# JianCao92/speaker-diarization

Hardware: AMD Instinct MI355X
Metric: diarized audio throughput (CD gw/BIC + CL hi/BIC) (higher is better)
Workload: dtype f64

## Files before the change

### include/spkd.h

```cpp
#ifndef SPKD_H
#define SPKD_H

#include <stddef.h>
#include <stdint.h>

#ifdef __cplusplus
extern "C" {
#endif

#define SPKD_ABI_VERSION 2
#define SPKD_DIM 39
#define SPKD_REC 820

typedef enum {
    SPKD_OK = 0,
    SPKD_EINVAL = 1,
    SPKD_EHIP = 2,
    SPKD_ENONFINITE = 3,
    SPKD_EOVERFLOW = 4,
    SPKD_ENOMEM = 5
} spkd_status;

typedef enum { SPKD_BIC = 0, SPKD_GLR = 1, SPKD_KL2 = 2, SPKD_KL2_PINV = 3 } spkd_kind;


typedef struct spkd_ctx spkd_ctx;

int spkd_abi_version(void);

spkd_status spkd_create(int device, void *stream, spkd_ctx **out);
spkd_status spkd_create_on_stream(int device, void *stream, spkd_ctx **out);
void spkd_destroy(spkd_ctx *ctx);
const char *spkd_last_error(const spkd_ctx *ctx);
spkd_status spkd_sync(spkd_ctx *ctx);

spkd_status spkd_malloc(spkd_ctx *ctx, size_t bytes, void **d_ptr);
spkd_status spkd_free(spkd_ctx *ctx, void *d_ptr);
spkd_status spkd_memcpy_h2d(spkd_ctx *ctx, void *d_dst, const void *h_src, size_t bytes);
spkd_status spkd_memcpy_d2h(spkd_ctx *ctx, void *h_dst, const void *d_src, size_t bytes);
spkd_status spkd_memcpy_d2d(spkd_ctx *ctx, void *d_dst, const void *d_src, size_t bytes);

enum {
    SPKD_T_CALL = 0, SPKD_T_CHUNK_STATS, SPKD_T_REDUCE_SETS, SPKD_T_PAIR_TERMS,
    SPKD_T_CLUSTER_PREP, SPKD_T_MATRIX, SPKD_T_AHC, SPKD_T_GW, SPKD_T_SW, SPKD_N_TIMERS
};
spkd_status spkd_last_kernel_ms(spkd_ctx *ctx, int which, float *ms);

spkd_status spkd_last_gw_items(spkd_ctx *ctx, int64_t *items);

spkd_status spkd_set_stats(spkd_ctx *ctx, const float *d_frames, int64_t n_frames,
                           const int64_t *h_range_begin, const int64_t *h_range_end,
                           const int32_t *h_range_set, int64_t n_ranges,
                           int64_t n_sets, double *d_stats);

#define SPKD_WANT_GLR 1
#define SPKD_WANT_KL2 2
#define SPKD_WANT_KL2_PINV 4
spkd_status spkd_pair_terms(spkd_ctx *ctx, const double *d_stats,
                            const int32_t *h_idx_a, const int32_t *h_idx_b,
                            int64_t n_pairs, int flags, double *h_terms);

spkd_status spkd_distance_matrix(spkd_ctx *ctx, int kind, double lambdac,
                                 const double *d_stats, int64_t n, double *d_matrix);

spkd_status spkd_cluster_in(spkd_ctx *ctx, const double *d_stats, int64_t n, int kind,
                            double lambdac, double threshold, int32_t *h_label,
                            double *h_dist, int64_t dist_cap, int64_t *h_dist_off,
                            int64_t *h_n_done, int64_t *h_n_clusters);

spkd_status spkd_distance_rows(spkd_ctx *ctx, int variant, int kind, double lambdac,
                               const double *d_stats, int64_t n, int64_t row_begin, int64_t row_end,
                               double *d_rows, double *h_stat_max, double *h_stat_min);

typedef struct {
    int32_t kind;
    int32_t trace;
    double lambdac;
    double threshold;
    double winsize;
    double winstep;
    double deltaws;
    double rate;
} spkd_cd_params;

typedef struct {
    int32_t turn;
    int32_t coarse;
    int64_t seq;
    double start, i, d;
    int64_t n1, n2;
} spkd_cand_log;

int64_t spkd_gw_event_capacity(int64_t turn_len, double rate);
int64_t spkd_gw_event_capacity_p(int64_t turn_len, const spkd_cd_params *params);
spkd_status spkd_gw(spkd_ctx *ctx, const float *d_frames, int64_t n_frames,
                    const int64_t *h_turn_begin, const int64_t *h_turn_end, int64_t n_turns,
                    const spkd_cd_params *params, const int64_t *h_ev_off,
                    int32_t *h_n_win, double *h_win_maxd, int32_t *h_win_det,
                    double *h_det_start, double *h_det_maxi, double *h_det_d,
                    double *h_final_start,
                    spkd_cand_log *h_log, int64_t log_cap, int64_t *h_log_count);

spkd_status spkd_gw_ex(spkd_ctx *ctx, const float *d_frames, int64_t n_frames,
                       const int64_t *h_turn_begin, const int64_t *h_turn_end, int64_t n_turns,
                       const spkd_cd_params *params, const int64_t *h_ev_off, int check_capacity,
                       int32_t *h_n_win, double *h_win_maxd, int32_t *h_win_det,
                       double *h_det_start, double *h_det_maxi, double *h_det_d,
                       double *h_final_start,
                       spkd_cand_log *h_log, int64_t log_cap, int64_t *h_log_count);

spkd_status spkd_gw_fused(spkd_ctx *ctx, const float *d_frames, int64_t n_frames,
                          const int64_t *h_turn_begin, const int64_t *h_turn_end, int64_t n_turns,
                          const spkd_cd_params *params, const int64_t *h_ev_off, int check_capacity,
                          int32_t *h_n_win, double *h_win_maxd, int32_t *h_win_det,
                          double *h_det_start, double *h_det_maxi, double *h_det_d,
                          double *h_final_start, double *d_seg_stats,
                          spkd_cand_log *h_log, int64_t log_cap, int64_t *h_log_count);

spkd_status spkd_gather_stats(spkd_ctx *ctx, const double *d_src, int64_t n_src,
                              const int64_t *h_src_index, const int64_t *h_dst_index,
                              int64_t n, int64_t n_dst, double *d_dst);

int64_t spkd_sw_window_count(int64_t turn_len, double winsize, double winstep);
spkd_status spkd_sw(spkd_ctx *ctx, const float *d_frames, int64_t n_frames,
                    const int64_t *h_turn_begin, const int64_t *h_turn_end, int64_t n_turns,
                    const spkd_cd_params *params, const int64_t *h_d_off, double *h_d);

enum { SPKD_AHC_AUTO = 0, SPKD_AHC_MONO = 1, SPKD_AHC_WIDE = 2 };

typedef struct {
    int32_t variant;
    int32_t kind;
    int32_t max_spk;
    int32_t path;
    double lambdac;
    double threshold;
} spkd_ahc_params;

spkd_status spkd_ahc(spkd_ctx *ctx, const double *d_stats, const int64_t *h_seg_off,
                     int64_t n_problems, const spkd_ahc_params *params,
                     int32_t *h_n_merges, int32_t *h_merge_a, int32_t *h_merge_b,
                     double *h_merge_d, double *h_stat_max, double *h_stat_min);

spkd_status spkd_ahc_matrix(spkd_ctx *ctx, const double *d_stats, int64_t n, const spkd_ahc_params *params,
                            const double *d_matrix, double stat_max_in, double stat_min_in,
                            int32_t *h_n_merges, int32_t *h_merge_a, int32_t *h_merge_b,
                            double *h_merge_d, double *h_stat_max, double *h_stat_min);

typedef struct {
    int32_t sample_rate, frame_rate, window_width, n_fft, n_mel, n_cep;
    int32_t cms_left, cms_right;
    int32_t delta_width[2];
    float pre_emph;
    float delta_norm[2];
} spkd_mfcc_params;
spkd_status spkd_mfcc(spkd_ctx *ctx, const int16_t *d_pcm, int64_t n_samples,
                      const spkd_mfcc_params *params, const float *h_melfb, const float *h_dct,
                      const float *h_mean, const float *h_scale, const float *h_transform,
                      float *d_features, int64_t *h_n_frames);

typedef struct {
    int32_t n_kernels, n_states, dim;
    const float *mean;
    const float *inv_var;
    const float *log_norm;
    const int32_t *state_off;
    const int32_t *kernel;
    const float *log_weight;
} spkd_gmm_params;
spkd_status spkd_gmm_loglik(spkd_ctx *ctx, const float *d_features, int64_t n_frames,
                            const spkd_gmm_params *params, float *d_scores);

void spkd_py2_roundtrip(double *h_values, int64_t n);
spkd_status spkd_labels_from_merges(int64_t n, int64_t n_merges, const int32_t *h_a,
                                    const int32_t *h_b, int32_t *h_labels);
spkd_status spkd_labels_from_merges_batch(int64_t n_problems, const int64_t *h_seg_off,
                                          const int32_t *h_n_merges, const int32_t *h_a,
                                          const int32_t *h_b, int32_t *h_labels);

spkd_status spkd_count_flags(const int32_t *h_flags, const int64_t *h_off, const int32_t *h_n,
                             int64_t n_groups, int32_t *h_out);

spkd_status spkd_gw_lines(int64_t n_turns, const int64_t *h_off, const int32_t *h_n_det,
                          const double *h_det_start, const double *h_det_maxi,
                          const double *h_final_start, const double *h_turn_start_s,
                          const double *h_turn_end_s, const int64_t *h_turn_begin,
                          const int64_t *h_turn_end, double rate, int text_contract,
                          int64_t n_lines, double *h_times, int64_t *h_frame_b,
                          int64_t *h_frame_e, int64_t *h_index, int32_t *h_line_turn);

spkd_status spkd_vad_viterbi(int64_t n_frames, int32_t n_states, const float *h_scores,
                             int32_t n_words, const int32_t *h_word_state, const double *h_stay,
                             const double *h_exit, const double *h_enter, int64_t *h_tok_frame,
                             int32_t *h_tok_word, int64_t *h_n_tokens, double *h_score);

#ifdef __cplusplus
}
#endif
#endif
```

### speaker-diarization_amd/csrc/spkd_hip.hip

```cpp
#include <hip/hip_runtime.h>

#include <algorithm>
#include <cmath>
#include <cstdio>
#include <cstdlib>
#include <cstring>
#include <string>
#include <atomic>
#include <thread>
#include <vector>

#include "../../include/spkd.h"
#include "spkd_cd.hpp"
#include "spkd_cluster.hpp"
#include "spkd_device.hpp"
#include "spkd_stats.hpp"
#include "spkd_mfcc.hpp"
#include "spkd_vad.hpp"

using namespace spkd;

namespace {
constexpr int N_SLOTS = 36;
}

struct spkd_ctx {
    int device = 0;
    hipStream_t stream = nullptr;
    bool own_stream = false;
    bool gw_lds_ok = false;
    int gw_waves = 0;
    unsigned long long init_keys[2] = {0ull, ~0ull};
    int step_waves = 0;
    int step_partners = 0;
    int64_t last_gw_items = 0;
    std::string err;
    int* d_err = nullptr;
    unsigned long long* d_counter = nullptr;
    hipEvent_t ev0 = nullptr, ev1 = nullptr;
    float last_ms = 0.f;
    hipEvent_t ka[SPKD_N_TIMERS] = {}, kb[SPKD_N_TIMERS] = {};
    bool kused[SPKD_N_TIMERS] = {};
    float kms[SPKD_N_TIMERS] = {};
    void* slot[N_SLOTS] = {};
    size_t slot_bytes[N_SLOTS] = {};
    void* pinv_ws = nullptr;
    double* pinv_cur = nullptr;
};

namespace {

spkd_status fail(spkd_ctx* c, spkd_status s, const std::string& msg) {
    if (c) c->err = msg;
    return s;
}

#define HIPCHK(c, call)                                                              \
    do {                                                                             \
        hipError_t e_ = (call);                                                      \
        if (e_ != hipSuccess)                                                        \
            return fail((c), SPKD_EHIP, std::string(#call) + ": " + hipGetErrorString(e_)); \
    } while (0)

#define TRY(expr) do { const spkd_status s_ = (expr); if (s_ != SPKD_OK) return s_; } while (0)

spkd_status scratch(spkd_ctx* c, int slot, size_t bytes, void** out) {
    if (bytes == 0) bytes = 16;
    if (c->slot_bytes[slot] < bytes) {
        if (c->slot[slot]) HIPCHK(c, hipFree(c->slot[slot]));
        c->slot[slot] = nullptr;
        c->slot_bytes[slot] = 0;
        size_t want = bytes + bytes / 4;
        hipError_t e = hipMalloc(&c->slot[slot], want);
        if (e != hipSuccess) {
            want = bytes;
            e = hipMalloc(&c->slot[slot], want);
        }
        if (e != hipSuccess) return fail(c, SPKD_ENOMEM, "scratch allocation failed");
        c->slot_bytes[slot] = want;
    }
    *out = c->slot[slot];
    return SPKD_OK;
}

template <class T>
spkd_status upload(spkd_ctx* c, int slot, const T* h, size_t n, T** d) {
    void* p = nullptr;
    TRY(scratch(c, slot, n * sizeof(T), &p));
    if (n) HIPCHK(c, hipMemcpyAsync(p, h, n * sizeof(T), hipMemcpyHostToDevice, c->stream));
    *d = (T*)p;
    return SPKD_OK;
}

struct Call {
    spkd_ctx* const c;
    spkd_status opened;
    int herr = 0;
    bool drained = false;
    explicit Call(spkd_ctx* ctx) : c(ctx) { opened = open(); }
    ~Call() { if (!drained) (void)hipStreamSynchronize(c->stream); }
    spkd_status open() {
        HIPCHK(c, hipSetDevice(c->device));
        for (int i = 0; i < SPKD_N_TIMERS; ++i) c->kused[i] = false;
        HIPCHK(c, hipMemsetAsync(c->d_err, 0, sizeof(int), c->stream));
        HIPCHK(c, hipEventRecord(c->ev0, c->stream));
        return SPKD_OK;
    }

    spkd_status finish() {
        HIPCHK(c, hipEventRecord(c->ev1, c->stream));
        HIPCHK(c, hipMemcpyAsync(&herr, c->d_err, sizeof(int), hipMemcpyDeviceToHost, c->stream));
        HIPCHK(c, hipStreamSynchronize(c->stream));
        drained = true;
        HIPCHK(c, hipEventElapsedTime(&c->last_ms, c->ev0, c->ev1));
        c->kms[0] = c->last_ms;
        for (int i = 1; i < SPKD_N_TIMERS; ++i)
            if (c->kused[i]) HIPCHK(c, hipEventElapsedTime(&c->kms[i], c->ka[i], c->kb[i]));
        if (herr & ERR_SWEEP) return fail(c, SPKD_EHIP, "internal error: growing-window sweep order");
        if (herr & 4) return fail(c, SPKD_EOVERFLOW, "device scratch capacity exceeded");
        if (herr & ERR_DEGENERATE_MERGE) return fail(c, SPKD_EINVAL, "degenerate merge: a diagonal cell was the minimum");
        if (herr & ERR_NONFINITE) return fail(c, SPKD_ENONFINITE, "array must not contain infs or NaNs");
        return SPKD_OK;
    }
};

spkd_status use_kind(spkd_ctx* c, int kind, int* base) {
    c->pinv_cur = nullptr;
    *base = kind;
    if (kind != SPKD_KL2_PINV) return SPKD_OK;
    *base = SPKD_KL2;
    if (!c->pinv_ws) {
        if (hipMalloc(&c->pinv_ws, PINV_WS_BYTES) != hipSuccess) {
            c->pinv_ws = nullptr;
            return fail(c, SPKD_ENOMEM, "pinv workspace allocation failed");
        }
        HIPCHK(c, hipMemsetAsync(c->pinv_ws, 0, PINV_LOCK_BYTES, c->stream));
    }
    c->pinv_cur = (double*)c->pinv_ws;
    return SPKD_OK;
}

struct Timer {
    spkd_ctx* const c;
    const int idx;
    Timer(spkd_ctx* ctx, int i) : c(ctx), idx(i) { (void)hipEventRecord(c->ka[idx], c->stream); }
    ~Timer() { (void)hipEventRecord(c->kb[idx], c->stream); c->kused[idx] = true; }
};

enum {
    S_CHUNKS = 0, S_SETOFF, S_PARTIAL, S_IDXA, S_IDXB, S_TERMS, S_TURNS, S_SNAP, S_CAND,
    S_EV_I32A, S_EV_I32B, S_EV_D0, S_EV_D1, S_EV_D2, S_EV_D3, S_EV_D4, S_LOG,
    S_AHC_STATS, S_AHC_LD, S_AHC_AUX, S_AHC_MAT, S_AHC_MISC, S_AHC_OUT, S_AHC_OFF, S_AHC_PROB, S_AHC_PACKED, S_MFCC_TAB, S_MFCC_STATIC,
    S_STEP_EXM, S_STEP_PKM, S_STEP_MISC, S_GMM_TAB, S_GMM_IDX, S_COUNT
};
static_assert(S_COUNT <= N_SLOTS, "scratch slot table too small");

}

extern "C" {

int spkd_abi_version(void) { return SPKD_ABI_VERSION; }

static spkd_status create_ctx(int device, void* stream, bool borrow, spkd_ctx** out) {
    if (!out) return SPKD_EINVAL;
    *out = nullptr;
    int count = 0;
    if (hipGetDeviceCount(&count) != hipSuccess || device < 0 || device >= count) return SPKD_EHIP;
    spkd_ctx* c = new spkd_ctx();
    c->device = device;
    if (hipSetDevice(device) != hipSuccess) { delete c; return SPKD_EHIP; }
    if (borrow) {
        c->stream = (hipStream_t)stream;
    } else {
        if (hipStreamCreateWithFlags(&c->stream, hipStreamDefault) != hipSuccess) { delete c; return SPKD_EHIP; }
        c->own_stream = true;
    }
    if (hipMalloc(&c->d_err, sizeof(int)) != hipSuccess ||
        hipMalloc(&c->d_counter, 2 * sizeof(unsigned long long)) != hipSuccess ||
        hipEventCreate(&c->ev0) != hipSuccess || hipEventCreate(&c->ev1) != hipSuccess) {
        spkd_destroy(c);
        return SPKD_EHIP;
    }
    for (int i = 0; i < SPKD_N_TIMERS; ++i)
        if (hipEventCreate(&c->ka[i]) != hipSuccess || hipEventCreate(&c->kb[i]) != hipSuccess) {
            spkd_destroy(c);
            return SPKD_EHIP;
        }
    int lds_max = 0;
    c->gw_lds_ok = hipDeviceGetAttribute(&lds_max, hipDeviceAttributeMaxSharedMemoryPerBlock, device) == hipSuccess &&
                   Gw<4>::LDS_BYTES <= lds_max &&
                   hipFuncSetAttribute((const void*)k_gw<8>, hipFuncAttributeMaxDynamicSharedMemorySize, Gw<8>::LDS_BYTES) == hipSuccess &&
                   hipFuncSetAttribute((const void*)k_gw<4>, hipFuncAttributeMaxDynamicSharedMemorySize, Gw<4>::LDS_BYTES) == hipSuccess &&
                   hipFuncSetAttribute((const void*)k_gw<2>, hipFuncAttributeMaxDynamicSharedMemorySize, Gw<2>::LDS_BYTES) == hipSuccess &&
                   hipFuncSetAttribute((const void*)k_gw<1>, hipFuncAttributeMaxDynamicSharedMemorySize, Gw<1>::LDS_BYTES) == hipSuccess;
    if (const char* e = getenv("SPKD_GW_WAVES")) c->gw_waves = atoi(e);
    if (const char* e = getenv("SPKD_STEP_WAVES")) { const int v = atoi(e); c->step_waves = (v == 4 || v == 8) ? v : 0; }
    if (const char* e = getenv("SPKD_STEP_PARTNERS")) { const int v = atoi(e); c->step_partners = (v == 3 || v == 7 || v == 15) ? v : 0; }
    *out = c;
    return SPKD_OK;
}

spkd_status spkd_create(int device, void* stream, spkd_ctx** out) {
    return create_ctx(device, stream, stream != nullptr, out);
}

spkd_status spkd_create_on_stream(int device, void* stream, spkd_ctx** out) {
    return create_ctx(device, stream, true, out);
}

void spkd_destroy(spkd_ctx* c) {
    if (!c) return;
    (void)hipSetDevice(c->device);
    if (c->stream) (void)hipStreamSynchronize(c->stream);
    for (int i = 0; i < N_SLOTS; ++i)
        if (c->slot[i]) (void)hipFree(c->slot[i]);
    if (c->d_err) (void)hipFree(c->d_err);
    if (c->pinv_ws) (void)hipFree(c->pinv_ws);
    if (c->d_counter) (void)hipFree(c->d_counter);
    if (c->ev0) (void)hipEventDestroy(c->ev0);
    if (c->ev1) (void)hipEventDestroy(c->ev1);
    for (int i = 0; i < SPKD_N_TIMERS; ++i) {
        if (c->ka[i]) (void)hipEventDestroy(c->ka[i]);
        if (c->kb[i]) (void)hipEventDestroy(c->kb[i]);
    }
    if (c->own_stream && c->stream) (void)hipStreamDestroy(c->stream);
    delete c;
}

const char* spkd_last_error(const spkd_ctx* c) { return c ? c->err.c_str() : "null context"; }

spkd_status spkd_sync(spkd_ctx* c) {
    if (!c) return SPKD_EINVAL;
    HIPCHK(c, hipStreamSynchronize(c->stream));
    return SPKD_OK;
}

spkd_status spkd_malloc(spkd_ctx* c, size_t bytes, void** d_ptr) {
    if (!c || !d_ptr) return SPKD_EINVAL;
    HIPCHK(c, hipSetDevice(c->device));
    hipError_t e = hipMalloc(d_ptr, bytes ? bytes : 16);
    if (e != hipSuccess) return fail(c, SPKD_ENOMEM, hipGetErrorString(e));
    return SPKD_OK;
}

spkd_status spkd_free(spkd_ctx* c, void* d_ptr) {
    if (!c) return SPKD_EINVAL;
    HIPCHK(c, hipFree(d_ptr));
    return SPKD_OK;
}

spkd_status spkd_memcpy_h2d(spkd_ctx* c, void* d_dst, const void* h_src, size_t bytes) {
    if (!c) return SPKD_EINVAL;
    HIPCHK(c, hipMemcpyAsync(d_dst, h_src, bytes, hipMemcpyHostToDevice, c->stream));
    HIPCHK(c, hipStreamSynchronize(c->stream));
    return SPKD_OK;
}

spkd_status spkd_memcpy_d2h(spkd_ctx* c, void* h_dst, const void* d_src, size_t bytes) {
    if (!c) return SPKD_EINVAL;
    HIPCHK(c, hipMemcpyAsync(h_dst, d_src, bytes, hipMemcpyDeviceToHost, c->stream));
    HIPCHK(c, hipStreamSynchronize(c->stream));
    return SPKD_OK;
}

spkd_status spkd_memcpy_d2d(spkd_ctx* c, void* d_dst, const void* d_src, size_t bytes) {
    if (!c) return SPKD_EINVAL;
    HIPCHK(c, hipMemcpyAsync(d_dst, d_src, bytes, hipMemcpyDeviceToDevice, c->stream));
    HIPCHK(c, hipStreamSynchronize(c->stream));
    return SPKD_OK;
}

spkd_status spkd_last_gw_items(spkd_ctx* c, int64_t* items) {
    if (!c || !items) return SPKD_EINVAL;
    *items = c->last_gw_items;
    return SPKD_OK;
}

spkd_status spkd_last_kernel_ms(spkd_ctx* c, int which, float* ms) {
    if (!c || !ms || which < 0 || which >= SPKD_N_TIMERS) return SPKD_EINVAL;
    *ms = c->kms[which];
    return SPKD_OK;
}

namespace {
spkd_status set_stats_launch(spkd_ctx* c, const float* d_frames, int64_t n_frames,
                             const int64_t* h_begin, const int64_t* h_end, const int32_t* h_set,
                             int64_t n_ranges, int64_t n_sets, double* d_stats,
                             std::vector<Chunk>& chunks, std::vector<int64_t>& set_off) {
    chunks.clear();
    set_off.assign((size_t)n_sets + 1, 0);
    int32_t prev = 0;
    for (int64_t r = 0; r < n_ranges; ++r) {
        const int64_t b = h_begin[r], e = h_end[r];
        const int32_t s = h_set[r];
        if (b < 0 || e < b || e > n_frames || s < prev || s >= n_sets)
            return fail(c, SPKD_EINVAL, "bad frame range or set id");
        prev = s;
        for (int64_t t = b; t < e; t += STATS_CHUNK) {
            Chunk ch;
            ch.begin = t;
            ch.len = (int32_t)std::min<int64_t>(STATS_CHUNK, e - t);
            ch.set = s;
            chunks.push_back(ch);
            set_off[(size_t)s + 1]++;
        }
    }
    for (int64_t s = 0; s < n_sets; ++s) set_off[(size_t)s + 1] += set_off[(size_t)s];
    Chunk* d_chunks = nullptr;
    int64_t* d_setoff = nullptr;
    void* d_partial = nullptr;
    TRY(upload(c, S_CHUNKS, chunks.data(), chunks.size(), &d_chunks));
    TRY(upload(c, S_SETOFF, set_off.data(), set_off.size(), &d_setoff));
    TRY(scratch(c, S_PARTIAL, chunks.size() * REC * sizeof(double), &d_partial));
    if (!chunks.empty()) {
        Timer t(c, SPKD_T_CHUNK_STATS);
        hipLaunchKernelGGL(k_chunk_stats, dim3((unsigned)chunks.size()), dim3(STATS_TPB), 0, c->stream,
                           d_frames, d_chunks, (double*)d_partial);
    }
    Timer t(c, SPKD_T_REDUCE_SETS);
    hipLaunchKernelGGL(k_reduce_sets, dim3((unsigned)n_sets), dim3(STATS_TPB), 0, c->stream,
                       (const double*)d_partial, d_setoff, d_stats);
    HIPCHK(c, hipGetLastError());
    return SPKD_OK;
}
}

spkd_status spkd_set_stats(spkd_ctx* c, const float* d_frames, int64_t n_frames,
                           const int64_t* h_begin, const int64_t* h_end, const int32_t* h_set,
                           int64_t n_ranges, int64_t n_sets, double* d_stats) {
    if (!c || !d_stats || n_sets < 0 || n_ranges < 0) return SPKD_EINVAL;
    if (n_sets == 0) return SPKD_OK;
    if (n_ranges > 0 && (!h_begin || !h_end || !h_set || !d_frames)) return fail(c, SPKD_EINVAL, "null range arrays");
    std::vector<Chunk> chunks;
    std::vector<int64_t> set_off;
    Call call(c);
    TRY(call.opened);
    TRY(set_stats_launch(c, d_frames, n_frames, h_begin, h_end, h_set, n_ranges, n_sets, d_stats, chunks, set_off));
    return call.finish();
}

spkd_status spkd_pair_terms(spkd_ctx* c, const double* d_stats, const int32_t* h_a, const int32_t* h_b,
                            int64_t n_pairs, int flags, double* h_terms) {
    if (!c || n_pairs < 0) return SPKD_EINVAL;
    if (n_pairs == 0) return SPKD_OK;
    if (!d_stats || !h_a || !h_b || !h_terms) return fail(c, SPKD_EINVAL, "null argument");
    if ((flags & SPKD_WANT_KL2) && (flags & SPKD_WANT_KL2_PINV))
        return fail(c, SPKD_EINVAL, "pair_terms: SPKD_WANT_KL2 and SPKD_WANT_KL2_PINV exclude each other");
    Call call(c);
    TRY(call.opened);
    int kind_unused;
    TRY(use_kind(c, (flags & SPKD_WANT_KL2_PINV) ? (int)SPKD_KL2_PINV : (int)SPKD_KL2, &kind_unused));
    if (flags & SPKD_WANT_KL2_PINV) flags = (flags & ~SPKD_WANT_KL2_PINV) | SPKD_WANT_KL2;
    int32_t *d_a = nullptr, *d_b = nullptr;
    void* d_terms = nullptr;
    TRY(upload(c, S_IDXA, h_a, (size_t)n_pairs, &d_a));
    TRY(upload(c, S_IDXB, h_b, (size_t)n_pairs, &d_b));
    TRY(scratch(c, S_TERMS, (size_t)n_pairs * 8 * sizeof(double), &d_terms));
    const unsigned blocks = (unsigned)((n_pairs + PT2_WAVES - 1) / PT2_WAVES);
    {
        Timer t(c, SPKD_T_PAIR_TERMS);
        hipLaunchKernelGGL(k_pair_terms, dim3(blocks), dim3(PT2_WAVES * WAVE), 0, c->stream,
                           d_stats, d_a, d_b, n_pairs, flags, (double*)d_terms, c->d_err, c->pinv_cur);
    }
    HIPCHK(c, hipGetLastError());
    HIPCHK(c, hipMemcpyAsync(h_terms, d_terms, (size_t)n_pairs * 8 * sizeof(double), hipMemcpyDeviceToHost, c->stream));
    return call.finish();
}

namespace {
struct AhcBuffers {
    double* ex;
    double* pk;
    double* ld;
    double* aux;
    double* mat;
    int64_t* seg_off;
    int64_t* mat_off;
    unsigned long long* smax;
    unsigned long long* smin;
};

unsigned long long host_dkey(double v) {
    unsigned long long b;
    std::memcpy(&b, &v, sizeof b);
    return (b >> 63) ? ~b : (b | 0x8000000000000000ull);
}

struct MatrixPlan {
    const double* d_init = nullptr;
    double init_max = NAN, init_min = NAN;
    int64_t row_begin = -1, row_end = -1;
};

spkd_status ahc_prepare(spkd_ctx* c, const double* d_stats, const int64_t* h_seg_off, int64_t n_prob,
                        int variant, int kind, double lambdac, AhcBuffers& B, int64_t& n_total,
                        std::vector<int64_t>& offs, std::vector<int32_t>& prob_of,
                        const MatrixPlan& plan = MatrixPlan()) {
    n_total = h_seg_off[n_prob];
    offs.clear();
    offs.insert(offs.end(), h_seg_off, h_seg_off + n_prob + 1);
    int64_t cells = 0;
    for (int64_t p = 0; p < n_prob; ++p) {
        const int64_t n = h_seg_off[p + 1] - h_seg_off[p];
        if (n < 0) return fail(c, SPKD_EINVAL, "seg_off must be non-decreasing");
        offs.push_back(cells);
        cells += n * n;
    }
    offs.push_back(cells);
    prob_of.assign((size_t)n_total, 0);
    for (int64_t p = 0; p < n_prob; ++p)
        for (int64_t r = h_seg_off[p]; r < h_seg_off[p + 1]; ++r) prob_of[(size_t)r] = (int32_t)p;
    int64_t grid_rows = 0;
    {
        const int X = 8;
        std::vector<std::vector<int32_t>> lists(X);
        if (plan.row_begin >= 0) {
            for (int64_t r = plan.row_begin; r < plan.row_end; ++r) lists[(size_t)((r - plan.row_begin) % X)].push_back((int32_t)r);
        } else if (n_prob >= X) {
            std::vector<int64_t> order((size_t)n_prob);
            for (int64_t p = 0; p < n_prob; ++p) order[(size_t)p] = p;
            std::stable_sort(order.begin(), order.end(), [&](int64_t a, int64_t b) {
                return h_seg_off[a + 1] - h_seg_off[a] > h_seg_off[b + 1] - h_seg_off[b];
            });
            double load[X] = {0, 0, 0, 0, 0, 0, 0, 0};
            for (int64_t p : order) {
                int x = 0;
                for (int i = 1; i < X; ++i) if (load[i] < load[x]) x = i;
                const double n = (double)(h_seg_off[p + 1] - h_seg_off[p]);
                load[x] += n * n;
                for (int64_t r = h_seg_off[p]; r < h_seg_off[p + 1]; ++r) lists[x].push_back((int32_t)r);
            }
        } else {
            for (int64_t r = 0; r < n_total; ++r) lists[(size_t)(r % X)].push_back((int32_t)r);
        }
        size_t longest = 0;
        for (auto& l : lists) longest = std::max(longest, l.size());
        grid_rows = (int64_t)longest * X;
        prob_of.resize((size_t)(n_total + grid_rows), -1);
        for (int x = 0; x < X; ++x)
            for (size_t i = 0; i < lists[x].size(); ++i) prob_of[(size_t)n_total + i * X + x] = lists[x][i];
    }
    int64_t* d_offs = nullptr;
    int32_t* d_prob = nullptr;
    TRY(upload(c, S_AHC_OFF, offs.data(), offs.size(), &d_offs));
    TRY(upload(c, S_AHC_PROB, prob_of.data(), prob_of.size(), &d_prob));
    B.seg_off = d_offs;
    B.mat_off = d_offs + n_prob + 1;
    void* p = nullptr;
    TRY(scratch(c, S_AHC_LD, (size_t)n_total * sizeof(double), &p));
    B.ld = (double*)p;
    TRY(scratch(c, S_AHC_AUX, (size_t)n_total * AUX * sizeof(double), &p));
    B.aux = (double*)p;
    TRY(scratch(c, S_AHC_MAT, (size_t)cells * sizeof(double), &p));
    B.mat = (double*)p;
    TRY(scratch(c, S_AHC_MISC, (size_t)n_prob * 2 * sizeof(unsigned long long), &p));
    B.smax = (unsigned long long*)p;
    B.smin = B.smax + n_prob;
    HIPCHK(c, hipMemsetAsync(B.smax, 0x00, (size_t)n_prob * sizeof(unsigned long long), c->stream));
    HIPCHK(c, hipMemsetAsync(B.smin, 0xff, (size_t)n_prob * sizeof(unsigned long long), c->stream));
    if (plan.d_init && n_prob == 1) {
        c->init_keys[0] = plan.init_max == plan.init_max ? host_dkey(plan.init_max) : 0ull;
        c->init_keys[1] = plan.init_min == plan.init_min ? host_dkey(plan.init_min) : ~0ull;
        HIPCHK(c, hipMemcpyAsync(B.smax, &c->init_keys[0], sizeof(unsigned long long), hipMemcpyHostToDevice, c->stream));
        HIPCHK(c, hipMemcpyAsync(B.smin, &c->init_keys[1], sizeof(unsigned long long), hipMemcpyHostToDevice, c->stream));
    }
    TRY(scratch(c, S_AHC_STATS, (size_t)n_total * QREC * sizeof(double), &p));
    B.ex = (double*)p;
    TRY(scratch(c, S_AHC_PACKED, (size_t)n_total * REC * sizeof(double), &p));
    B.pk = (double*)p;
    if (n_total > 0) {
        hipLaunchKernelGGL(k_to_quadrec, dim3((unsigned)n_total), dim3(256), 0, c->stream, d_stats, n_total, B.ex);
        HIPCHK(c, hipMemcpyAsync(B.pk, d_stats, (size_t)n_total * REC * sizeof(double), hipMemcpyDeviceToDevice, c->stream));
        const int64_t per_block = kind == SPKD_KL2 ? PT_WAVES : 4 * PT_WAVES;
        const unsigned blocks = (unsigned)((n_total + per_block - 1) / per_block);
        {
            Timer t(c, SPKD_T_CLUSTER_PREP);
            hipLaunchKernelGGL(k_cluster_prep, dim3(blocks), dim3(PT_WAVES * WAVE), 0, c->stream,
                               (const double*)B.ex, n_total, kind, B.ld, B.aux, c->d_err, c->pinv_cur);
        }
        auto kmat = kind == SPKD_GLR ? k_matrix<true> : k_matrix<false>;
        if (plan.d_init) {
            HIPCHK(c, hipMemcpyAsync(B.mat, plan.d_init, (size_t)cells * sizeof(double), hipMemcpyDeviceToDevice, c->stream));
        } else if (grid_rows > 0) {
            Timer t(c, SPKD_T_MATRIX);
            hipLaunchKernelGGL(kmat, dim3((unsigned)grid_rows), dim3(MX_WAVES * WAVE), 0, c->stream,
                               (const double*)B.ex, (const double*)B.pk, (const int64_t*)B.seg_off, (const int32_t*)d_prob,
                               (const int32_t*)d_prob + n_total, variant, kind, lambdac,
                               (const double*)B.ld, (const double*)B.aux, B.mat, (const int64_t*)B.mat_off,
                               B.smax, B.smin, c->d_err);
        }
    }
    HIPCHK(c, hipGetLastError());
    return SPKD_OK;
}

double key_to_double(unsigned long long k, bool is_max) {
    if (is_max ? (k == 0ull) : (k == ~0ull)) return std::nan("");
    unsigned long long b = (k >> 63) ? (k & 0x7fffffffffffffffull) : ~k;
    double v;
    std::memcpy(&v, &b, sizeof v);
    return v;
}
}

spkd_status spkd_distance_matrix(spkd_ctx* c, int kind, double lambdac, const double* d_stats,
                                 int64_t n, double* d_matrix) {
    if (!c || n < 0 || kind < 0 || kind > 3) return SPKD_EINVAL;
    if (n == 0) return SPKD_OK;
    if (!d_stats || !d_matrix) return fail(c, SPKD_EINVAL, "null argument");
    const int64_t seg_off[2] = {0, n};
    AhcBuffers B;
    int64_t n_total = 0;
    std::vector<int64_t> offs;
    std::vector<int32_t> prob_of;
    Call call(c);
    TRY(call.opened);
    TRY(use_kind(c, kind, &kind));
    TRY(ahc_prepare(c, d_stats, seg_off, 1, 1, kind, lambdac, B, n_total, offs, prob_of));
    HIPCHK(c, hipMemcpyAsync(d_matrix, B.mat, (size_t)n * n * sizeof(double), hipMemcpyDeviceToDevice, c->stream));
    return call.finish();
}

spkd_status spkd_cluster_in(spkd_ctx* c, const double* d_stats, int64_t n, int kind, double lambdac, double threshold,
                            int32_t* h_label, double* h_dist, int64_t dist_cap, int64_t* h_dist_off,
                            int64_t* h_n_done, int64_t* h_n_clusters) {
    if (!c || n < 0 || dist_cap < 0 || kind < 0 || kind > 3) return SPKD_EINVAL;
    if (h_n_done) *h_n_done = 0;
    if (h_n_clusters) *h_n_clusters = 0;
    if (n == 0) return SPKD_OK;
    if (!d_stats || !h_label || !h_dist_off || !h_n_done || !h_n_clusters || (dist_cap > 0 && !h_dist))
        return fail(c, SPKD_EINVAL, "null argument");
    long long done2[2] = {0, 0};
    Call call(c);
    TRY(call.opened);
    TRY(use_kind(c, kind, &kind));
    void *p_ex = nullptr, *p_ld = nullptr, *p_aux = nullptr, *p_cex = nullptr, *p_cpk = nullptr, *p_misc = nullptr, *p_dist = nullptr;
    const size_t nn = (size_t)n;
    TRY(scratch(c, S_AHC_STATS, nn * QREC * sizeof(double), &p_ex));
    TRY(scratch(c, S_AHC_LD, nn * sizeof(double), &p_ld));
    TRY(scratch(c, S_AHC_AUX, nn * AUX * sizeof(double), &p_aux));
    TRY(scratch(c, S_STEP_EXM, nn * QREC * sizeof(double), &p_cex));
    TRY(scratch(c, S_STEP_PKM, nn * REC * sizeof(double), &p_cpk));
    const size_t misc_bytes = (2 + AUX) * nn * sizeof(double) + (nn + 1 + 2) * sizeof(long long) + nn * sizeof(int32_t) + 64;
    TRY(scratch(c, S_STEP_MISC, misc_bytes, &p_misc));
    TRY(scratch(c, S_AHC_MAT, (size_t)std::max<int64_t>(dist_cap, 1) * sizeof(double), &p_dist));
    double* clu_ld = (double*)p_misc;
    double* tmp = clu_ld + nn;
    double* clu_aux = tmp + nn;
    long long* d_off = (long long*)(clu_aux + nn * AUX);
    long long* d_done = d_off + nn + 1;
    int32_t* d_label = (int32_t*)(d_done + 2);
    HIPCHK(c, hipMemsetAsync(d_done, 0, 2 * sizeof(long long), c->stream));
    hipLaunchKernelGGL(k_to_quadrec, dim3((unsigned)n), dim3(256), 0, c->stream, d_stats, n, (double*)p_ex);
    {
        const int64_t per_block = 4 * PT_WAVES;
        const unsigned blocks = (unsigned)((n + per_block - 1) / per_block);
        {
            Timer t(c, SPKD_T_CLUSTER_PREP);
            hipLaunchKernelGGL(k_cluster_prep, dim3(blocks), dim3(PT_WAVES * WAVE), 0, c->stream,
                               (const double*)p_ex, n, kind == SPKD_KL2 ? (int)SPKD_BIC : kind, (double*)p_ld, (double*)p_aux, c->d_err,
                               c->pinv_cur);
        }
        if (kind == SPKD_KL2) {
            void* p_ld2 = nullptr;
            TRY(scratch(c, S_AHC_OUT, nn * sizeof(double), &p_ld2));
            const unsigned blocks1 = (unsigned)((n + PT_WAVES - 1) / PT_WAVES);
            hipLaunchKernelGGL(k_cluster_prep, dim3(blocks1), dim3(PT_WAVES * WAVE), 0, c->stream,
                               (const double*)p_ex, n, (int)SPKD_KL2, (double*)p_ld2, (double*)p_aux, c->d_err, c->pinv_cur);
        }
    }
    auto kin = kind == SPKD_GLR ? k_cluster_in<true> : k_cluster_in<false>;
    {
        Timer t(c, SPKD_T_AHC);
        hipLaunchKernelGGL(kin, dim3(1), dim3(CIN_TPB), 0, c->stream,
                           (const double*)p_ex, d_stats, (const double*)p_ld, (const double*)p_aux, (long long)n, kind, lambdac, threshold,
                           (double*)p_cex, (double*)p_cpk, clu_ld, clu_aux, tmp, d_label, (double*)p_dist, (long long)dist_cap,
                           d_off, d_done, c->d_err, c->pinv_cur);
    }
    HIPCHK(c, hipGetLastError());
    HIPCHK(c, hipMemcpyAsync(done2, d_done, sizeof done2, hipMemcpyDeviceToHost, c->stream));
    HIPCHK(c, hipMemcpyAsync(h_label, d_label, nn * sizeof(int32_t), hipMemcpyDeviceToHost, c->stream));
    HIPCHK(c, hipMemcpyAsync(h_dist_off, d_off, (nn + 1) * sizeof(long long), hipMemcpyDeviceToHost, c->stream));
    if (dist_cap > 0)
        HIPCHK(c, hipMemcpyAsync(h_dist, p_dist, (size_t)dist_cap * sizeof(double), hipMemcpyDeviceToHost, c->stream));
    const spkd_status st = call.finish();
    *h_n_done = done2[0];
    *h_n_clusters = done2[1];
    return st;
}

spkd_status spkd_distance_rows(spkd_ctx* c, int variant, int kind, double lambdac, const double* d_stats,
                               int64_t n, int64_t row_begin, int64_t row_end, double* d_rows,
                               double* h_stat_max, double* h_stat_min) {
    if (!c || n < 0 || kind < 0 || kind > 3 || (variant != 1 && variant != 2)) return SPKD_EINVAL;
    if (row_begin < 0 || row_end < row_begin || row_end > n) return fail(c, SPKD_EINVAL, "distance_rows: bad row block");
    if (h_stat_max) *h_stat_max = std::nan("");
    if (h_stat_min) *h_stat_min = std::nan("");
    if (n == 0 || row_end == row_begin) return SPKD_OK;
    if (!d_stats || !d_rows) return fail(c, SPKD_EINVAL, "null argument");
    const int64_t seg_off[2] = {0, n};
    AhcBuffers B;
    int64_t n_total = 0;
    std::vector<int64_t> offs;
    std::vector<int32_t> prob_of;
    MatrixPlan plan;
    plan.row_begin = row_begin;
    plan.row_end = row_end;
    unsigned long long keys[2] = {0ull, ~0ull};
    Call call(c);
    TRY(call.opened);
    TRY(use_kind(c, kind, &kind));
    TRY(ahc_prepare(c, d_stats, seg_off, 1, variant, kind, lambdac, B, n_total, offs, prob_of, plan));
    HIPCHK(c, hipMemcpyAsync(d_rows, B.mat + row_begin * n, (size_t)(row_end - row_begin) * n * sizeof(double),
                             hipMemcpyDeviceToDevice, c->stream));
    HIPCHK(c, hipMemcpyAsync(&keys[0], B.smax, sizeof(unsigned long long), hipMemcpyDeviceToHost, c->stream));
    HIPCHK(c, hipMemcpyAsync(&keys[1], B.smin, sizeof(unsigned long long), hipMemcpyDeviceToHost, c->stream));
    const spkd_status st = call.finish();
    if (h_stat_max) *h_stat_max = key_to_double(keys[0], true);
    if (h_stat_min) *h_stat_min = key_to_double(keys[1], false);
    return st;
}

namespace {
spkd_status ahc_impl(spkd_ctx* c, const double* d_stats, const int64_t* h_seg_off, int64_t n_prob,
                     const spkd_ahc_params* P, const MatrixPlan& plan, int32_t* h_n_merges, int32_t* h_merge_a,
                     int32_t* h_merge_b, double* h_merge_d, double* h_stat_max, double* h_stat_min) {
    if (!c || !P || n_prob < 0) return SPKD_EINVAL;
    if (n_prob == 0) return SPKD_OK;
    if (!d_stats || !h_seg_off || !h_n_merges || !h_merge_a || !h_merge_b || !h_merge_d ||
        !h_stat_max || !h_stat_min)
        return fail(c, SPKD_EINVAL, "null argument");
    if ((P->variant != 1 && P->variant != 2) || P->kind < 0 || P->kind > 3)
        return fail(c, SPKD_EINVAL, "bad variant / kind");
    for (int64_t p = 0; p < n_prob; ++p)
        if (h_seg_off[p + 1] - h_seg_off[p] < 1) return fail(c, SPKD_EINVAL, "empty clustering problem");
    int64_t n_max = 0;
    for (int64_t p = 0; p < n_prob; ++p) n_max = std::max<int64_t>(n_max, h_seg_off[p + 1] - h_seg_off[p]);
    if (n_max > AHC_MAX_N) return fail(c, SPKD_EINVAL, "clustering problem larger than 65536 records");
    int path = P->path;
    if (path != SPKD_AHC_MONO && path != SPKD_AHC_WIDE) path = n_prob <= 64 ? SPKD_AHC_WIDE : SPKD_AHC_MONO;
    const size_t lds = (size_t)(n_max + 4) * sizeof(int32_t);
    if (path == SPKD_AHC_MONO && lds > 150 * 1024) path = SPKD_AHC_WIDE;
    if (path == SPKD_AHC_WIDE && n_max > STEP_MAX_N)
        return fail(c, SPKD_EINVAL, "clustering problem larger than 16384 records (wide merge loop)");
    AhcBuffers B;
    int64_t n_total = 0;
    std::vector<int64_t> offs;
    std::vector<int32_t> prob_of;
    std::vector<unsigned long long> kmax((size_t)n_prob), kmin((size_t)n_prob);
    std::vector<double> fmax((size_t)n_prob), fmin((size_t)n_prob);
    Call call(c);
    TRY(call.opened);
    spkd_ahc_params Pk = *P;
    TRY(use_kind(c, P->kind, &Pk.kind));
    P = &Pk;
    TRY(ahc_prepare(c, d_stats, h_seg_off, n_prob, P->variant, P->kind, P->lambdac, B, n_total, offs, prob_of, plan));
    void* op = nullptr;
    const size_t out_bytes = (size_t)n_total * (6 * sizeof(int32_t) + 3 * sizeof(double)) +
                             (size_t)n_prob * (sizeof(int32_t) + 2 * sizeof(double)) + 64;
    TRY(scratch(c, S_AHC_OUT, out_bytes, &op));
    double* d_merge_d = (double*)op;
    double* d_tmp = d_merge_d + n_total;
    double* d_rmin = d_tmp + n_total;
    double* d_fmax = d_rmin + n_total;
    double* d_fmin = d_fmax + n_prob;
    int32_t* d_a = (int32_t*)(d_fmin + n_prob);
    int32_t* d_b = d_a + n_total;
    int32_t* d_alive = d_b + n_total;
    int32_t* d_rcache = d_alive + n_total;
    int32_t* d_n = d_rcache + 3 * n_total;
    if (path == SPKD_AHC_MONO) {
        auto kahc = P->kind == SPKD_GLR ? k_ahc<true> : k_ahc<false>;
        if (lds > 48 * 1024)
            (void)hipFuncSetAttribute((const void*)kahc, hipFuncAttributeMaxDynamicSharedMemorySize, (int)lds);
        Timer t(c, SPKD_T_AHC);
        hipLaunchKernelGGL(kahc, dim3((unsigned)n_prob), dim3(AHC_TPB), lds, c->stream,
                           B.ex, B.pk, (const int64_t*)B.seg_off, P->variant, P->kind, P->max_spk, P->lambdac,
                           P->threshold, B.ld, B.aux, B.mat, (const int64_t*)B.mat_off, d_alive, d_tmp,
                           d_rmin, d_rcache, d_n, d_a, d_b, d_merge_d, B.smax, B.smin, d_fmax, d_fmin, c->d_err,
                           c->pinv_cur);
    } else {
        StepArrays Q;
        void *pm = nullptr, *pe = nullptr, *pp = nullptr;
        const size_t nt = (size_t)n_total;
        const size_t misc_bytes = nt * 2 * sizeof(StepSel) + nt * sizeof(double) + nt * sizeof(unsigned long long) +
                                  (size_t)2 * n_prob * sizeof(StepState) + nt * sizeof(int32_t) + 64;
        TRY(scratch(c, S_STEP_MISC, misc_bytes, &pm));
        TRY(scratch(c, S_STEP_EXM, nt * QREC * sizeof(double), &pe));
        TRY(scratch(c, S_STEP_PKM, nt * REC * sizeof(double), &pp));
        Q.ex = B.ex; Q.pk = B.pk; Q.exm = (double*)pe; Q.pkm = (double*)pp;
        Q.sel2 = (StepSel*)pm;
        Q.cnt = (double*)(Q.sel2 + 2 * nt);
        Q.sw = (unsigned long long*)(Q.cnt + nt);
        Q.state2 = (StepState*)(Q.sw + nt);
        Q.death = (int32_t*)(Q.state2 + 2 * n_prob);
        Q.n_total = n_total;
        Q.n_prob = (int32_t)n_prob;
        const int step_waves = c->step_waves ? c->step_waves : (n_max > STEP_WIDE_FROM ? 8 : 4);
        const bool glr_k = P->kind == SPKD_GLR;
        using StepKernel = decltype(&k_ahc_step<false, 4, 3>);
        StepKernel kvar[3];
        if (step_waves == 8) {
            kvar[0] = glr_k ? k_ahc_step<true, 8, 3> : k_ahc_step<false, 8, 3>;
            kvar[1] = glr_k ? k_ahc_step<true, 8, 7> : k_ahc_step<false, 8, 7>;
            kvar[2] = glr_k ? k_ahc_step<true, 8, STEP_PARTNERS> : k_ahc_step<false, 8, STEP_PARTNERS>;
        } else {
            kvar[0] = glr_k ? k_ahc_step<true, 4, 3> : k_ahc_step<false, 4, 3>;
            kvar[1] = glr_k ? k_ahc_step<true, 4, 7> : k_ahc_step<false, 4, 7>;
            kvar[2] = glr_k ? k_ahc_step<true, 4, STEP_PARTNERS> : k_ahc_step<false, 4, STEP_PARTNERS>;
        }
        auto sp_of_round = [&](int64_t partners) -> int {
            if (c->step_partners) return c->step_partners;
            const int64_t free_cus = 255;
            if (partners * n_prob <= 3 * free_cus) return 3;
            if (partners * n_prob <= 7 * free_cus) return 7;
            return STEP_PARTNERS;
        };
        const size_t nch_max = (size_t)((n_max + WAVE - 1) / WAVE);
        const size_t step_lds = ((size_t)2 * n_max + nch_max + 2) * sizeof(int32_t) + nch_max * sizeof(unsigned long long);
        if (step_lds + 20 * 1024 > 48 * 1024)
            for (int v = 0; v < 3; ++v)
                (void)hipFuncSetAttribute((const void*)kvar[v], hipFuncAttributeMaxDynamicSharedMemorySize, (int)step_lds);
        Timer t(c, SPKD_T_AHC);
        const unsigned row_blocks = (unsigned)((n_max + AHC_WAVES - 1) / AHC_WAVES);
        hipLaunchKernelGGL(k_step_init, dim3(row_blocks, (unsigned)n_prob), dim3(AHC_TPB), 0, c->stream,
                           (const int64_t*)B.seg_off, (const double*)B.mat, (const int64_t*)B.mat_off, Q);
        for (int64_t it = 1; it < n_max; ++it) {
            const int64_t partners = n_max - it - 1;
            const int step_sp = sp_of_round(partners);
            StepKernel kstep = kvar[step_sp == 3 ? 0 : (step_sp == 7 ? 1 : 2)];
            const unsigned blocks = (unsigned)std::max<int64_t>(1, (partners + step_sp - 1) / step_sp) + 1;
            hipLaunchKernelGGL(kstep, dim3(blocks, (unsigned)n_prob), dim3(step_waves * WAVE), step_lds, c->stream,
                               (int)it, (const int64_t*)B.seg_off, P->variant, P->kind, P->max_spk, P->lambdac,
                               P->threshold, B.ld, B.aux, B.mat, (const int64_t*)B.mat_off, Q, d_a, d_b, d_merge_d,
                               B.smax, B.smin, c->d_err, c->pinv_cur);
        }
        hipLaunchKernelGGL(k_step_final, dim3((unsigned)n_prob), dim3(AHC_TPB), 0, c->stream,
                           (int)(n_max - 1), (const int64_t*)B.seg_off, (const double*)B.mat, (const int64_t*)B.mat_off,
                           Q, d_n, d_fmax, d_fmin);
    }
    HIPCHK(c, hipGetLastError());
    HIPCHK(c, hipMemcpyAsync(h_n_merges, d_n, (size_t)n_prob * sizeof(int32_t), hipMemcpyDeviceToHost, c->stream));
    HIPCHK(c, hipMemcpyAsync(h_merge_a, d_a, (size_t)n_total * sizeof(int32_t), hipMemcpyDeviceToHost, c->stream));
    HIPCHK(c, hipMemcpyAsync(h_merge_b, d_b, (size_t)n_total * sizeof(int32_t), hipMemcpyDeviceToHost, c->stream));
    HIPCHK(c, hipMemcpyAsync(h_merge_d, d_merge_d, (size_t)n_total * sizeof(double), hipMemcpyDeviceToHost, c->stream));
    HIPCHK(c, hipMemcpyAsync(kmax.data(), B.smax, (size_t)n_prob * sizeof(unsigned long long), hipMemcpyDeviceToHost, c->stream));
    HIPCHK(c, hipMemcpyAsync(kmin.data(), B.smin, (size_t)n_prob * sizeof(unsigned long long), hipMemcpyDeviceToHost, c->stream));
    HIPCHK(c, hipMemcpyAsync(fmax.data(), d_fmax, (size_t)n_prob * sizeof(double), hipMemcpyDeviceToHost, c->stream));
    HIPCHK(c, hipMemcpyAsync(fmin.data(), d_fmin, (size_t)n_prob * sizeof(double), hipMemcpyDeviceToHost, c->stream));
    const spkd_status st = call.finish();
    for (int64_t p = 0; p < n_prob; ++p) {
        if (P->variant == 1) {
            h_stat_max[p] = key_to_double(kmax[(size_t)p], true);
            h_stat_min[p] = key_to_double(kmin[(size_t)p], false);
        } else {
            h_stat_max[p] = fmax[(size_t)p];
            h_stat_min[p] = fmin[(size_t)p];
        }
    }
    return st;
}
}

spkd_status spkd_ahc(spkd_ctx* c, const double* d_stats, const int64_t* h_seg_off, int64_t n_prob,
                     const spkd_ahc_params* P, int32_t* h_n_merges, int32_t* h_merge_a,
                     int32_t* h_merge_b, double* h_merge_d, double* h_stat_max, double* h_stat_min) {
    return ahc_impl(c, d_stats, h_seg_off, n_prob, P, MatrixPlan(), h_n_merges, h_merge_a, h_merge_b, h_merge_d,
                    h_stat_max, h_stat_min);
}

spkd_status spkd_ahc_matrix(spkd_ctx* c, const double* d_stats, int64_t n, const spkd_ahc_params* P,
                            const double* d_matrix, double stat_max_in, double stat_min_in,
                            int32_t* h_n_merges, int32_t* h_merge_a, int32_t* h_merge_b, double* h_merge_d,
                            double* h_stat_max, double* h_stat_min) {
    if (!c || n < 1) return SPKD_EINVAL;
    if (!d_matrix) return fail(c, SPKD_EINVAL, "ahc_matrix: null matrix");
    const int64_t seg_off[2] = {0, n};
    MatrixPlan plan;
    plan.d_init = d_matrix;
    plan.init_max = stat_max_in;
    plan.init_min = stat_min_in;
    return ahc_impl(c, d_stats, seg_off, 1, P, plan, h_n_merges, h_merge_a, h_merge_b, h_merge_d, h_stat_max, h_stat_min);
}

int64_t spkd_gw_event_capacity(int64_t turn_len, double rate) {
    if (turn_len < 0 || !(rate >= 10.0)) return -1;
    return (int64_t)((double)turn_len / (0.2 * rate)) + 8;
}

int64_t spkd_gw_event_capacity_p(int64_t turn_len, const spkd_cd_params* P) {
    if (turn_len < 0 || !P || !(P->rate >= 10.0) || !(P->winstep >= 1.0)) return -1;
    const double step = std::min(0.2 * P->rate, std::min(0.5 * P->rate, P->winstep));
    return (int64_t)((double)turn_len / step) + 8;
}

int64_t spkd_sw_window_count(int64_t turn_len, double winsize, double winstep) {
    if (!(winstep >= 1.0) || !(winsize >= 1.0)) return -1;
    int64_t w = 0;
    for (double s = 0; s + 2 * winsize <= (double)turn_len; s += winstep) ++w;
    return w;
}

namespace {
spkd_status build_turns(spkd_ctx* c, int64_t n_frames, const int64_t* hb, const int64_t* he, int64_t n_turns,
                        const spkd_cd_params* P, const int64_t* h_off, bool gw, std::vector<TurnDesc>& turns,
                        int64_t& n_cand) {
    n_cand = 0;
    turns.resize((size_t)n_turns);
    for (int64_t t = 0; t < n_turns; ++t) {
        if (hb[t] < 0 || he[t] < hb[t] || he[t] > n_frames) return fail(c, SPKD_EINVAL, "bad turn range");
        TurnDesc& T = turns[(size_t)t];
        T.begin = hb[t];
        T.len = he[t] - hb[t];
        T.cand_off = n_cand;
        T.cand_cap = gw ? (int64_t)((double)T.len / (P->rate / 10)) + (int64_t)(2 * (P->rate / 10)) + 16 : 0;
        n_cand += T.cand_cap;
        T.ev_off = h_off[t];
        T.ev_cap = h_off[t + 1] - h_off[t];
        T.id = t;
        if (T.ev_cap < 0) return fail(c, SPKD_EINVAL, "offsets must be non-decreasing");
    }
    if (gw) std::stable_sort(turns.begin(), turns.end(), [](const TurnDesc& a, const TurnDesc& b) { return a.len > b.len; });
    return SPKD_OK;
}
}

namespace {
constexpr int64_t GW_WAVE_PER_TURN_FROM = 4096;
constexpr int64_t GW_EIGHT_WAVES_UP_TO = 256;
spkd_status gw_impl(spkd_ctx* c, const float* d_frames, int64_t n_frames, const int64_t* hb,
                    const int64_t* he, int64_t n_turns, const spkd_cd_params* P, const int64_t* h_ev_off,
                    int check_capacity, int32_t* h_n_win, double* h_win_maxd, int32_t* h_win_det,
                    double* h_det_start, double* h_det_maxi, double* h_det_d, double* h_final_start,
                    double* d_seg_stats, spkd_cand_log* h_log, int64_t log_cap, int64_t* h_log_count) {
    if (!c || !P || n_turns < 0) return SPKD_EINVAL;
    if (h_log_count) *h_log_count = 0;
    if (n_turns == 0) return SPKD_OK;
    if (!d_frames || !hb || !he || !h_ev_off || !h_n_win || !h_win_maxd || !h_win_det || !h_det_start ||
        !h_det_maxi || !h_det_d || !h_final_start)
        return fail(c, SPKD_EINVAL, "null argument");
    if (P->kind < 0 || P->kind > 3) return fail(c, SPKD_EINVAL, "gw: bad kind");
    if (!(P->rate >= 10.0) || !(P->winsize >= 1.0) || !(P->winstep >= 1.0))
        return fail(c, SPKD_EINVAL, "gw: rate >= 10, winsize >= 1 frame and winstep >= 1 frame required");
    if (log_cap < 0 || (log_cap > 0 && !h_log)) return fail(c, SPKD_EINVAL, "gw: log capacity without a log buffer");
    if (!c->gw_lds_ok) return fail(c, SPKD_EHIP, "gw: the kernel's dynamic LDS size was not admitted on this device");
    std::vector<TurnDesc> turns;
    int64_t n_cand;
    TRY(build_turns(c, n_frames, hb, he, n_turns, P, h_ev_off, true, turns, n_cand));
    for (int64_t t = 0; check_capacity && t < n_turns; ++t)
        if (turns[(size_t)t].ev_cap < spkd_gw_event_capacity_p(turns[(size_t)t].len, P))
            return fail(c, SPKD_EINVAL, "gw: event capacity too small, see spkd_gw_event_capacity_p");
    unsigned long long cnt2[2] = {0ull, 0ull};
    Call call(c);
    TRY(call.opened);
    spkd_cd_params Pk = *P;
    TRY(use_kind(c, P->kind, &Pk.kind));
    P = &Pk;
    const int64_t n_ev = h_ev_off[n_turns];
    TurnDesc* d_turns = nullptr;
    void *d_snap = nullptr, *d_cand = nullptr, *d_i32a = nullptr, *d_i32b = nullptr, *d_d0 = nullptr, *d_d1 = nullptr,
         *d_d2 = nullptr, *d_d3 = nullptr, *d_d4 = nullptr, *d_log = nullptr;
    TRY(upload(c, S_TURNS, turns.data(), turns.size(), &d_turns));
    TRY(scratch(c, S_SNAP, (size_t)n_cand * REC * sizeof(double), &d_snap));
    TRY(scratch(c, S_CAND, (size_t)n_cand * 4 * sizeof(double), &d_cand));
    TRY(scratch(c, S_EV_I32A, (size_t)n_turns * sizeof(int32_t), &d_i32a));
    TRY(scratch(c, S_EV_I32B, (size_t)n_ev * sizeof(int32_t), &d_i32b));
    TRY(scratch(c, S_EV_D0, (size_t)n_ev * sizeof(double), &d_d0));
    TRY(scratch(c, S_EV_D1, (size_t)n_ev * sizeof(double), &d_d1));
    TRY(scratch(c, S_EV_D2, (size_t)n_ev * sizeof(double), &d_d2));
    TRY(scratch(c, S_EV_D3, (size_t)n_ev * sizeof(double), &d_d3));
    TRY(scratch(c, S_EV_D4, (size_t)n_turns * sizeof(double), &d_d4));
    TRY(scratch(c, S_LOG, (size_t)std::max<int64_t>(log_cap, 1) * sizeof(spkd_cand_log), &d_log));
    if (!d_turns || !d_snap || !d_cand || !d_i32a || !d_i32b || !d_d0 || !d_d1 || !d_d2 || !d_d3 || !d_d4 ||
        !d_log || !c->d_counter || !c->d_err)
        return fail(c, SPKD_EHIP, "gw: a device scratch buffer is missing");
    HIPCHK(c, hipMemsetAsync(c->d_counter, 0, 2 * sizeof(unsigned long long), c->stream));
    int nw = c->gw_waves;
    if (nw != 1 && nw != 2 && nw != 4 && nw != 8)
        nw = n_turns >= GW_WAVE_PER_TURN_FROM ? 1 : (n_turns <= GW_EIGHT_WAVES_UP_TO ? 8 : 4);
#define SPKD_GW_LAUNCH(NW_)                                                                                     \
    hipLaunchKernelGGL(k_gw<NW_>, dim3((unsigned)n_turns), dim3(Gw<NW_>::TPB), Gw<NW_>::LDS_BYTES, c->stream, \
                       d_frames, (const TurnDesc*)d_turns, *P, (double*)d_snap, (double*)d_cand,               \
                       (int32_t*)d_i32a, (double*)d_d0, (int32_t*)d_i32b, (double*)d_d1, (double*)d_d2,        \
                       (double*)d_d3, (double*)d_d4, d_seg_stats, (spkd_cand_log*)d_log, (long long)log_cap,   \
                       c->d_counter, c->d_err, c->pinv_cur)
    {
        Timer t(c, SPKD_T_GW);
        if (nw == 1) SPKD_GW_LAUNCH(1); else if (nw == 2) SPKD_GW_LAUNCH(2);
        else if (nw == 8) SPKD_GW_LAUNCH(8); else SPKD_GW_LAUNCH(4);
    }
#undef SPKD_GW_LAUNCH
    HIPCHK(c, hipGetLastError());
    unsigned long long& cnt = cnt2[0];
    HIPCHK(c, hipMemcpyAsync(h_n_win, d_i32a, (size_t)n_turns * sizeof(int32_t), hipMemcpyDeviceToHost, c->stream));
    HIPCHK(c, hipMemcpyAsync(h_win_maxd, d_d0, (size_t)n_ev * sizeof(double), hipMemcpyDeviceToHost, c->stream));
    HIPCHK(c, hipMemcpyAsync(h_win_det, d_i32b, (size_t)n_ev * sizeof(int32_t), hipMemcpyDeviceToHost, c->stream));
    HIPCHK(c, hipMemcpyAsync(h_det_start, d_d1, (size_t)n_ev * sizeof(double), hipMemcpyDeviceToHost, c->stream));
    HIPCHK(c, hipMemcpyAsync(h_det_maxi, d_d2, (size_t)n_ev * sizeof(double), hipMemcpyDeviceToHost, c->stream));
    HIPCHK(c, hipMemcpyAsync(h_det_d, d_d3, (size_t)n_ev * sizeof(double), hipMemcpyDeviceToHost, c->stream));
    HIPCHK(c, hipMemcpyAsync(h_final_start, d_d4, (size_t)n_turns * sizeof(double), hipMemcpyDeviceToHost, c->stream));
    HIPCHK(c, hipMemcpyAsync(cnt2, c->d_counter, sizeof cnt2, hipMemcpyDeviceToHost, c->stream));
    const spkd_status st = call.finish();
    c->last_gw_items = (int64_t)cnt2[1];
    if (h_log_count) *h_log_count = (int64_t)cnt;
    if (h_log && log_cap > 0 && cnt > 0) {
        const size_t ncopy = (size_t)std::min<int64_t>((int64_t)cnt, log_cap);
        HIPCHK(c, hipMemcpy(h_log, d_log, ncopy * sizeof(spkd_cand_log), hipMemcpyDeviceToHost));
    }
    if (st == SPKD_OK && (int64_t)cnt > log_cap && h_log)
        return fail(c, SPKD_EOVERFLOW, "candidate log too small");
    return st;
}
}

spkd_status spkd_gw(spkd_ctx* c, const float* d_frames, int64_t n_frames, const int64_t* hb,
                    const int64_t* he, int64_t n_turns, const spkd_cd_params* P, const int64_t* h_ev_off,
                    int32_t* h_n_win, double* h_win_maxd, int32_t* h_win_det, double* h_det_start,
                    double* h_det_maxi, double* h_det_d, double* h_final_start, spkd_cand_log* h_log,
                    int64_t log_cap, int64_t* h_log_count) {
    return gw_impl(c, d_frames, n_frames, hb, he, n_turns, P, h_ev_off, 1, h_n_win, h_win_maxd, h_win_det,
                   h_det_start, h_det_maxi, h_det_d, h_final_start, nullptr, h_log, log_cap, h_log_count);
}

spkd_status spkd_gw_ex(spkd_ctx* c, const float* d_frames, int64_t n_frames, const int64_t* hb,
                       const int64_t* he, int64_t n_turns, const spkd_cd_params* P, const int64_t* h_ev_off,
                       int check_capacity, int32_t* h_n_win, double* h_win_maxd, int32_t* h_win_det,
                       double* h_det_start, double* h_det_maxi, double* h_det_d, double* h_final_start,
                       spkd_cand_log* h_log, int64_t log_cap, int64_t* h_log_count) {
    return gw_impl(c, d_frames, n_frames, hb, he, n_turns, P, h_ev_off, check_capacity, h_n_win, h_win_maxd,
                   h_win_det, h_det_start, h_det_maxi, h_det_d, h_final_start, nullptr, h_log, log_cap,
                   h_log_count);
}

spkd_status spkd_gw_fused(spkd_ctx* c, const float* d_frames, int64_t n_frames, const int64_t* hb,
                          const int64_t* he, int64_t n_turns, const spkd_cd_params* P, const int64_t* h_ev_off,
                          int check_capacity, int32_t* h_n_win, double* h_win_maxd, int32_t* h_win_det,
                          double* h_det_start, double* h_det_maxi, double* h_det_d, double* h_final_start,
                          double* d_seg_stats, spkd_cand_log* h_log, int64_t log_cap, int64_t* h_log_count) {
    if (c && !d_seg_stats) return fail(c, SPKD_EINVAL, "gw_fused: null statistics buffer");
    return gw_impl(c, d_frames, n_frames, hb, he, n_turns, P, h_ev_off, check_capacity, h_n_win, h_win_maxd,
                   h_win_det, h_det_start, h_det_maxi, h_det_d, h_final_start, d_seg_stats, h_log, log_cap,
                   h_log_count);
}

namespace {
__global__ __launch_bounds__(256) void k_gather_records(const double* __restrict__ src, const int64_t* __restrict__ si,
                                                        const int64_t* __restrict__ di, int64_t n,
                                                        double* __restrict__ dst) {
    const int64_t i = blockIdx.x;
    if (i >= n) return;
    const double2* s = reinterpret_cast<const double2*>(src + si[i] * REC);
    double2* d = reinterpret_cast<double2*>(dst + (di ? di[i] : i) * REC);
    for (int e = threadIdx.x; e < REC / 2; e += 256) d[e] = s[e];
}
}

spkd_status spkd_gather_stats(spkd_ctx* c, const double* d_src, int64_t n_src, const int64_t* h_src_index,
                              const int64_t* h_dst_index, int64_t n, int64_t n_dst, double* d_dst) {
    if (!c || n < 0) return SPKD_EINVAL;
    if (n == 0) return SPKD_OK;
    if (!d_src || !h_src_index || !d_dst) return fail(c, SPKD_EINVAL, "null argument");
    for (int64_t i = 0; i < n; ++i) {
        if (h_src_index[i] < 0 || h_src_index[i] >= n_src) return fail(c, SPKD_EINVAL, "gather: source index out of range");
        const int64_t d = h_dst_index ? h_dst_index[i] : i;
        if (d < 0 || d >= n_dst) return fail(c, SPKD_EINVAL, "gather: destination index out of range");
    }
    Call call(c);
    TRY(call.opened);
    int64_t *d_si = nullptr, *d_di = nullptr;
    TRY(upload(c, S_IDXA, h_src_index, (size_t)n, &d_si));
    if (h_dst_index) TRY(upload(c, S_IDXB, h_dst_index, (size_t)n, &d_di));
    hipLaunchKernelGGL(k_gather_records, dim3((unsigned)n), dim3(256), 0, c->stream, d_src,
                       (const int64_t*)d_si, (const int64_t*)d_di, n, d_dst);
    HIPCHK(c, hipGetLastError());
    return call.finish();
}

namespace {
__global__ __launch_bounds__(256) void k_take_pair_distance(const double* __restrict__ mat, int64_t n, double* __restrict__ out) {
    const int64_t p = (int64_t)blockIdx.x * 256 + threadIdx.x;
    if (p < n) out[p] = mat[4 * p + 1];
}
}

spkd_status spkd_sw(spkd_ctx* c, const float* d_frames, int64_t n_frames, const int64_t* hb,
                    const int64_t* he, int64_t n_turns, const spkd_cd_params* P, const int64_t* h_d_off,
                    double* h_d) {
    if (!c || !P || n_turns < 0) return SPKD_EINVAL;
    if (n_turns == 0) return SPKD_OK;
    if (!d_frames || !hb || !he || !h_d_off || !h_d) return fail(c, SPKD_EINVAL, "null argument");
    if (P->kind < 0 || P->kind > 3) return fail(c, SPKD_EINVAL, "bad kind");
    if (!(P->winsize >= 1.0) || !(P->winstep >= 1.0)) return fail(c, SPKD_EINVAL, "sw: window and step must be >= 1 frame");
    const int64_t n_d = h_d_off[n_turns];
    std::vector<int64_t> rb, re;
    std::vector<int32_t> rs;
    rb.reserve((size_t)(2 * n_d)); re.reserve((size_t)(2 * n_d)); rs.reserve((size_t)(2 * n_d));
    const int64_t wsz = (int64_t)P->winsize;
    for (int64_t t = 0; t < n_turns; ++t) {
        if (hb[t] < 0 || he[t] < hb[t] || he[t] > n_frames) return fail(c, SPKD_EINVAL, "bad turn range");
        const int64_t len = he[t] - hb[t];
        const int64_t W = spkd_sw_window_count(len, P->winsize, P->winstep);
        if (h_d_off[t + 1] - h_d_off[t] != W) return fail(c, SPKD_EINVAL, "sw: offsets do not match spkd_sw_window_count");
        for (int64_t w = 0; w < W; ++w) {
            const int64_t a = hb[t] + (int64_t)((double)w * P->winstep);
            const int32_t s0 = (int32_t)(2 * (h_d_off[t] + w));
            rb.push_back(a); re.push_back(a + wsz); rs.push_back(s0);
            rb.push_back(a + wsz); re.push_back(a + 2 * wsz); rs.push_back(s0 + 1);
        }
    }
    if (n_d == 0) return SPKD_OK;
    if (2 * n_d > 0x7fffffffLL) return fail(c, SPKD_EINVAL, "sw: too many windows in one call");
    std::vector<Chunk> chunks;
    std::vector<int64_t> set_off, offs;
    std::vector<int32_t> prob_of;
    Call call(c);
    TRY(call.opened);
    spkd_cd_params Pk = *P;
    TRY(use_kind(c, P->kind, &Pk.kind));
    P = &Pk;
    void *d_rec = nullptr, *d_out = nullptr;
    TRY(scratch(c, S_SNAP, (size_t)(2 * n_d) * REC * sizeof(double), &d_rec));
    TRY(scratch(c, S_EV_D0, (size_t)n_d * sizeof(double), &d_out));
    {
        Timer t(c, SPKD_T_SW);
        TRY(set_stats_launch(c, d_frames, n_frames, rb.data(), re.data(), rs.data(), 2 * n_d, 2 * n_d, (double*)d_rec,
                             chunks, set_off));
        std::vector<int64_t> seg_off((size_t)n_d + 1);
        for (int64_t w = 0; w <= n_d; ++w) seg_off[(size_t)w] = 2 * w;
        AhcBuffers B;
        int64_t n_total = 0;
        TRY(ahc_prepare(c, (const double*)d_rec, seg_off.data(), n_d, 1, P->kind, P->lambdac, B, n_total, offs, prob_of));
        hipLaunchKernelGGL(k_take_pair_distance, dim3((unsigned)((n_d + 255) / 256)), dim3(256), 0, c->stream,
                           (const double*)B.mat, n_d, (double*)d_out);
    }
    HIPCHK(c, hipGetLastError());
    HIPCHK(c, hipMemcpyAsync(h_d, d_out, (size_t)n_d * sizeof(double), hipMemcpyDeviceToHost, c->stream));
    return call.finish();
}

spkd_status spkd_mfcc(spkd_ctx* c, const int16_t* d_pcm, int64_t n_samples, const spkd_mfcc_params* P,
                      const float* h_melfb, const float* h_dct, const float* h_mean, const float* h_scale,
                      const float* h_transform, float* d_features, int64_t* h_n_frames) {
    if (!c || !P || !h_n_frames) return SPKD_EINVAL;
    *h_n_frames = 0;
    if (n_samples < 0 || !h_melfb || !h_dct || !h_mean || !h_scale || !h_transform)
        return fail(c, SPKD_EINVAL, "mfcc: null argument");
    if ((P->window_width != MF_WIN && P->window_width != MF_WIN_VAD) || P->n_fft != MF_NFFT || P->n_mel != MF_MEL ||
        P->n_cep != MF_CEP || P->frame_rate <= 0 || P->sample_rate <= 0 || P->sample_rate % P->frame_rate != 0)
        return fail(c, SPKD_EINVAL, "mfcc: this build does 400- or 256-sample windows, a 512-point transform, 21 mel bins, 12 cepstra");
    if (P->cms_left < 0 || P->cms_right < 0 || P->cms_left + P->cms_right > 1024 || P->delta_width[0] < 1 ||
        P->delta_width[0] > 2 || P->delta_width[1] < 1 || P->delta_width[1] > 2 || !(P->delta_norm[0] > 0.f) ||
        !(P->delta_norm[1] > 0.f))
        return fail(c, SPKD_EINVAL, "mfcc: unsupported mean-subtraction window or delta parameters");
    const int hop = P->sample_rate / P->frame_rate;
    if (hop < 1) return fail(c, SPKD_EINVAL, "mfcc: frame rate above the sample rate");
    const int span = MP_FR + 2 * MP_HALO;
    const size_t lds = (size_t)((span + P->cms_left + P->cms_right) * MF_STATIC + 2 * span * MF_STATIC +
                                MP_FR * MF_DIM + MF_DIM * MF_DIM) * sizeof(float);
    if (lds > 60 * 1024) return fail(c, SPKD_EINVAL, "mfcc: mean-subtraction window too wide for the LDS tile");
    const int64_t T = n_samples / hop;
    *h_n_frames = T;
    if (T == 0) return SPKD_OK;
    if (!d_pcm || !d_features) return fail(c, SPKD_EINVAL, "mfcc: null device buffer");
    std::vector<float> tab;
    tab.insert(tab.end(), h_melfb, h_melfb + MF_MEL * MF_BINS);
    tab.insert(tab.end(), h_dct, h_dct + MF_CEP * MF_MEL);
    tab.insert(tab.end(), h_mean, h_mean + MF_DIM);
    tab.insert(tab.end(), h_scale, h_scale + MF_DIM);
    tab.insert(tab.end(), h_transform, h_transform + MF_DIM * MF_DIM);
    Call call(c);
    TRY(call.opened);
    float* d_tab = nullptr;
    void* d_static = nullptr;
    TRY(upload(c, S_MFCC_TAB, tab.data(), tab.size(), &d_tab));
    TRY(scratch(c, S_MFCC_STATIC, (size_t)T * MF_STATIC * sizeof(float), &d_static));
    const float* d_fb = d_tab;
    const float* d_dct = d_fb + MF_MEL * MF_BINS;
    const float* d_mean = d_dct + MF_CEP * MF_MEL;
    const float* d_scale = d_mean + MF_DIM;
    const float* d_tr = d_scale + MF_DIM;
    if (P->window_width == MF_WIN)
        hipLaunchKernelGGL(k_mfcc_static<MF_WIN>, dim3((unsigned)((T + MF_FR - 1) / MF_FR)), dim3(MF_TPB), 0, c->stream,
                           d_pcm, (long long)n_samples, (long long)T, hop, P->pre_emph, d_fb, d_dct, (float*)d_static);
    else
        hipLaunchKernelGGL(k_mfcc_static<MF_WIN_VAD>, dim3((unsigned)((T + MF_FR - 1) / MF_FR)), dim3(MF_TPB), 0,
                           c->stream, d_pcm, (long long)n_samples, (long long)T, hop, P->pre_emph, d_fb, d_dct,
                           (float*)d_static);
    hipLaunchKernelGGL(k_mfcc_post, dim3((unsigned)((T + MP_FR - 1) / MP_FR)), dim3(MF_TPB), lds, c->stream,
                       (const float*)d_static, (long long)T, P->cms_left, P->cms_right, P->delta_width[0],
                       P->delta_norm[0], P->delta_width[1], P->delta_norm[1], d_mean, d_scale, d_tr, d_features);
    if (hipGetLastError() != hipSuccess) return fail(c, SPKD_EHIP, "mfcc: kernel launch failed");
    return call.finish();
}

spkd_status spkd_gmm_loglik(spkd_ctx* c, const float* d_features, int64_t n_frames, const spkd_gmm_params* P,
                            float* d_scores) {
    if (!c || !P) return SPKD_EINVAL;
    const int K = P->n_kernels, S = P->n_states;
    if (P->dim != GM_DIM || K < 1 || K > GM_MAX_K || S < 1 || S > GM_MAX_S || n_frames < 0)
        return fail(c, SPKD_EINVAL, "gmm_loglik: dim must be 39, 1 <= kernels <= 256, 1 <= states <= 16");
    if (!P->mean || !P->inv_var || !P->log_norm || !P->state_off || !P->kernel || !P->log_weight)
        return fail(c, SPKD_EINVAL, "gmm_loglik: null model array");
    if (P->state_off[0] != 0) return fail(c, SPKD_EINVAL, "gmm_loglik: state_off[0] must be 0");
    for (int s = 0; s < S; ++s)
        if (P->state_off[s + 1] < P->state_off[s] || P->state_off[s + 1] - P->state_off[s] > K)
            return fail(c, SPKD_EINVAL, "gmm_loglik: state_off must be non-decreasing, at most 256 kernels a state");
    const int nnz = P->state_off[S];
    for (int j = 0; j < nnz; ++j) {
        const float lw = P->log_weight[j];
        if (P->kernel[j] < 0 || P->kernel[j] >= K || std::isnan(lw) || lw == INFINITY)
            return fail(c, SPKD_EINVAL, "gmm_loglik: kernel index out of range or log weight NaN / +inf");
    }
    for (int64_t i = 0; i < (int64_t)K * GM_DIM; ++i)
        if (!std::isfinite(P->mean[i]) || !std::isfinite(P->inv_var[i]) || !(P->inv_var[i] > 0.f))
            return fail(c, SPKD_EINVAL, "gmm_loglik: means must be finite, inverse variances finite and positive");
    for (int k = 0; k < K; ++k)
        if (!std::isfinite(P->log_norm[k])) return fail(c, SPKD_EINVAL, "gmm_loglik: non-finite normalising constant");
    if (n_frames == 0) return SPKD_OK;
    if (!d_features || !d_scores) return fail(c, SPKD_EINVAL, "gmm_loglik: null device buffer");
    const int64_t n_blocks = (n_frames + GM_TPB - 1) / GM_TPB;
    if (n_blocks > 0x7fffffffLL) return fail(c, SPKD_EINVAL, "gmm_loglik: too many frames in one call");
    std::vector<float> tab;
    tab.insert(tab.end(), P->mean, P->mean + (size_t)K * GM_DIM);
    tab.insert(tab.end(), P->inv_var, P->inv_var + (size_t)K * GM_DIM);
    tab.insert(tab.end(), P->log_norm, P->log_norm + K);
    tab.insert(tab.end(), P->log_weight, P->log_weight + nnz);
    std::vector<int32_t> idx(P->state_off, P->state_off + S + 1);
    idx.insert(idx.end(), P->kernel, P->kernel + nnz);
    Call call(c);
    TRY(call.opened);
    float* d_tab = nullptr;
    int32_t* d_idx = nullptr;
    TRY(upload(c, S_GMM_TAB, tab.data(), tab.size(), &d_tab));
    TRY(upload(c, S_GMM_IDX, idx.data(), idx.size(), &d_idx));
    const float* d_mean = d_tab;
    const float* d_iv = d_mean + (size_t)K * GM_DIM;
    const float* d_c = d_iv + (size_t)K * GM_DIM;
    const float* d_lw = d_c + K;
    hipLaunchKernelGGL(k_gmm_loglik, dim3((unsigned)n_blocks), dim3(GM_TPB), 0, c->stream, d_features,
                       (long long)n_frames, d_mean, d_iv, d_c, (const int*)d_idx, (const int*)(d_idx + S + 1), d_lw,
                       S, d_scores);
    if (hipGetLastError() != hipSuccess) return fail(c, SPKD_EHIP, "gmm_loglik: kernel launch failed");
    return call.finish();
}

static const double kPow10[23] = {1e0, 1e1, 1e2, 1e3, 1e4, 1e5, 1e6, 1e7, 1e8, 1e9, 1e10, 1e11,
                                  1e12, 1e13, 1e14, 1e15, 1e16, 1e17, 1e18, 1e19, 1e20, 1e21, 1e22};
static const uint64_t kPow10u[20] = {1ull, 10ull, 100ull, 1000ull, 10000ull, 100000ull, 1000000ull,
                                     10000000ull, 100000000ull, 1000000000ull, 10000000000ull,
                                     100000000000ull, 1000000000000ull, 10000000000000ull,
                                     100000000000000ull, 1000000000000000ull, 10000000000000000ull,
                                     100000000000000000ull, 1000000000000000000ull,
                                     10000000000000000000ull};

static bool roundtrip_fast(double x, double* out) {
    if (!(x >= 1e-3 && x < 1e11)) return false;
    int e10 = (int)std::floor(std::log10(x));
    if (e10 < -3) e10 = -3;
    if (e10 >= 0) { if (x < kPow10[e10]) --e10; else if (e10 + 1 <= 22 && x >= kPow10[e10 + 1]) ++e10; }
    else { if (x * kPow10[-e10] < 1.0) --e10; else if (x * kPow10[-e10 - 1] >= 1.0) ++e10; }
    if (e10 < -3 || e10 > 10) return false;
    int s = 11 - e10;
    int k;
    const double fr = std::frexp(x, &k);
    const uint64_t m = (uint64_t)std::ldexp(fr, 53);
    k -= 53;
    unsigned __int128 prod = (unsigned __int128)m * kPow10u[s];
    uint64_t q;
    if (k >= 0) {
        if (k > 20) return false;
        q = (uint64_t)(prod << k);
    } else {
        const int sh = -k;
        if (sh >= 120) return false;
        const unsigned __int128 one = 1;
        const unsigned __int128 fl = prod >> sh;
        const unsigned __int128 remn = prod & ((one << sh) - 1);
        const unsigned __int128 half = one << (sh - 1);
        q = (uint64_t)fl;
        if (remn > half || (remn == half && (q & 1))) ++q;
    }
    if (q >= 1000000000000ull) {
        if (q != 1000000000000ull) return false;
        q = 100000000000ull;
        s -= 1;
    } else if (q < 100000000000ull) {
        return false;
    }
    *out = s >= 0 ? (double)q / kPow10[s] : (double)q * kPow10[-s];
    return true;
}

static void roundtrip_range(double* v, int64_t lo, int64_t hi) {
    char buf[64];
    for (int64_t i = lo; i < hi; ++i) {
        double r;
        if (roundtrip_fast(v[i], &r)) { v[i] = r; continue; }
        std::snprintf(buf, sizeof buf, "%.12g", v[i]);
        v[i] = std::strtod(buf, nullptr);
    }
}

void spkd_py2_roundtrip(double* v, int64_t n) {
    const int64_t kMinPerThread = 8192;
    int nthreads = (int)std::min<int64_t>(8, n / kMinPerThread);
    if (nthreads <= 1) { roundtrip_range(v, 0, n); return; }
    std::vector<std::thread> pool;
    const int64_t step = (n + nthreads - 1) / nthreads;
    for (int t = 0; t < nthreads; ++t) {
        const int64_t lo = t * step, hi = std::min<int64_t>(n, lo + step);
        if (lo < hi) pool.emplace_back(roundtrip_range, v, lo, hi);
    }
    for (auto& th : pool) th.join();
}

spkd_status spkd_labels_from_merges(int64_t n, int64_t n_merges, const int32_t* h_a, const int32_t* h_b,
                                    int32_t* h_labels) {
    if (n < 0 || n_merges < 0 || (n > 0 && !h_labels) || (n_merges > 0 && (!h_a || !h_b))) return SPKD_EINVAL;
    std::vector<int32_t> ids((size_t)n), parent((size_t)n);
    for (int64_t i = 0; i < n; ++i) ids[(size_t)i] = parent[(size_t)i] = (int32_t)i;
    int64_t m = n;
    for (int64_t k = 0; k < n_merges; ++k) {
        const int32_t a = h_a[k], b = h_b[k];
        if (a < 0 || b <= a || b >= m) return SPKD_EINVAL;
        parent[(size_t)ids[(size_t)b]] = ids[(size_t)a];
        ids.erase(ids.begin() + b);
        --m;
    }
    std::vector<int32_t> where((size_t)n, -1);
    for (int64_t p = 0; p < m; ++p) where[(size_t)ids[(size_t)p]] = (int32_t)p;
    for (int64_t i = 0; i < n; ++i) {
        int32_t r = (int32_t)i;
        while (parent[(size_t)r] != r) r = parent[(size_t)r];
        int32_t c = (int32_t)i;
        while (parent[(size_t)c] != r) { const int32_t nx = parent[(size_t)c]; parent[(size_t)c] = r; c = nx; }
        h_labels[i] = where[(size_t)r] + 1;
    }
    return SPKD_OK;
}

spkd_status spkd_count_flags(const int32_t* h_flags, const int64_t* h_off, const int32_t* h_n, int64_t n_groups,
                             int32_t* h_out) {
    if (n_groups < 0 || (n_groups > 0 && (!h_flags || !h_off || !h_n || !h_out))) return SPKD_EINVAL;
    for (int64_t g = 0; g < n_groups; ++g) {
        if (h_n[g] < 0 || h_off[g] < 0) return SPKD_EINVAL;
        const int32_t* f = h_flags + h_off[g];
        int32_t c = 0;
        for (int32_t i = 0; i < h_n[g]; ++i) c += f[i] != 0;
        h_out[g] = c;
    }
    return SPKD_OK;
}

#pragma clang fp contract(off)
spkd_status spkd_gw_lines(int64_t n_turns, const int64_t* h_off, const int32_t* h_n_det, const double* h_det_start,
                          const double* h_det_maxi, const double* h_final_start, const double* h_turn_start_s,
                          const double* h_turn_end_s, const int64_t* h_turn_begin, const int64_t* h_turn_end,
                          double rate, int text_contract, int64_t n_lines, double* h_times, int64_t* h_frame_b,
                          int64_t* h_frame_e, int64_t* h_index, int32_t* h_line_turn) {
    if (n_turns < 0 || n_lines < 0) return SPKD_EINVAL;
    if (n_turns > 0 && (!h_off || !h_n_det || !h_det_start || !h_det_maxi || !h_final_start || !h_turn_start_s ||
                        !h_turn_end_s || !h_turn_begin || !h_turn_end || !h_times))
        return SPKD_EINVAL;
    int64_t i = 0;
    for (int64_t t = 0; t < n_turns; ++t) {
        const int64_t nd = h_n_det[t];
        if (nd < 0 || i + nd + 1 > n_lines) return SPKD_EINVAL;
        const double ls = h_turn_start_s[t], le = h_turn_end_s[t];
        for (int64_t j = 0; j <= nd; ++j, ++i) {
            const bool tail = j == nd;
            double fs, fe;
            if (tail) {
                fs = h_final_start[t];
                h_times[2 * i] = fs / rate + ls;
                h_times[2 * i + 1] = ((le - ls) * rate) / rate + ls;
                fe = 0.0;
            } else {
                fs = h_det_start[h_off[t] + j];
                fe = fs + h_det_maxi[h_off[t] + j];
                h_times[2 * i] = fs / rate + ls;
                h_times[2 * i + 1] = fe / rate + ls;
            }
            if (h_frame_b) h_frame_b[i] = h_turn_begin[t] + (int64_t)fs;
            if (h_frame_e) h_frame_e[i] = tail ? h_turn_end[t] : h_turn_begin[t] + (int64_t)fe;
            if (h_index) h_index[i] = h_off[t] + j;
            if (h_line_turn) h_line_turn[i] = (int32_t)t;
        }
    }
    if (i != n_lines) return SPKD_EINVAL;
    if (text_contract) spkd_py2_roundtrip(h_times, 2 * n_lines);
    return SPKD_OK;
}

spkd_status spkd_vad_viterbi(int64_t n_frames, int32_t n_states, const float* h_scores, int32_t n_words,
                             const int32_t* h_word_state, const double* h_stay, const double* h_exit,
                             const double* h_enter, int64_t* h_tok_frame, int32_t* h_tok_word, int64_t* h_n_tokens,
                             double* h_score) {
    if (!h_n_tokens || !h_score || n_frames < 0 || n_states < 1 || n_states > GM_MAX_S || n_words < 1 ||
        n_words > GM_MAX_S || !h_word_state || !h_stay || !h_exit || !h_enter)
        return SPKD_EINVAL;
    *h_n_tokens = 0;
    *h_score = -INFINITY;
    for (int32_t j = 0; j < n_words; ++j)
        if (h_word_state[j] < 0 || h_word_state[j] >= n_states) return SPKD_EINVAL;
    if (n_frames == 0) return SPKD_OK;
    if (!h_scores || !h_tok_frame || !h_tok_word) return SPKD_EINVAL;
    const int W = n_words;
    std::vector<int8_t> back((size_t)n_frames * W);
    double d[GM_MAX_S], nd[GM_MAX_S], obs[GM_MAX_S];
    for (int64_t t = 0; t < n_frames; ++t) {
        bool all_ninf = true;
        for (int j = 0; j < W; ++j) {
            const double o = (double)h_scores[t * n_states + h_word_state[j]];
            obs[j] = std::isnan(o) ? -INFINITY : o;
            all_ninf = all_ninf && obs[j] == -INFINITY;
        }
        if (all_ninf)
            for (int j = 0; j < W; ++j) obs[j] = 0.0;
        if (t == 0) {
            for (int j = 0; j < W; ++j) { d[j] = h_enter[j] + obs[j]; back[(size_t)j] = -1; }
            continue;
        }
        double best = d[0] + h_exit[0];
        int bi = 0;
        for (int i = 1; i < W; ++i) {
            const double v = d[i] + h_exit[i];
            if (v > best) { best = v; bi = i; }
        }
        for (int j = 0; j < W; ++j) {
            const double stay = d[j] + h_stay[j], sw = best + h_enter[j];
            int8_t& b = back[(size_t)t * W + j];
            if (stay >= sw) { nd[j] = stay + obs[j]; b = -1; }
            else { nd[j] = sw + obs[j]; b = (int8_t)bi; }
        }
        for (int j = 0; j < W; ++j) d[j] = nd[j];
    }
    int j = 0;
    for (int i = 1; i < W; ++i)
        if (d[i] > d[j]) j = i;
    *h_score = d[j];
    int64_t n = 0;
    for (int64_t t = n_frames - 1; t >= 0; --t) {
        const int8_t b = back[(size_t)t * W + j];
        if (t == 0 || b >= 0) { h_tok_frame[n] = t; h_tok_word[n] = j; ++n; }
        if (t > 0 && b >= 0) j = b;
    }
    std::reverse(h_tok_frame, h_tok_frame + n);
    std::reverse(h_tok_word, h_tok_word + n);
    *h_n_tokens = n;
    return SPKD_OK;
}

spkd_status spkd_labels_from_merges_batch(int64_t n_problems, const int64_t* h_seg_off, const int32_t* h_n_merges,
                                          const int32_t* h_a, const int32_t* h_b, int32_t* h_labels) {
    if (n_problems < 0 || (n_problems > 0 && (!h_seg_off || !h_n_merges || !h_a || !h_b || !h_labels)))
        return SPKD_EINVAL;
    std::atomic<int> bad{0};
    auto work = [&](int64_t lo, int64_t hi) {
        for (int64_t p = lo; p < hi; ++p) {
            const int64_t o = h_seg_off[p];
            if (spkd_labels_from_merges(h_seg_off[p + 1] - o, h_n_merges[p], h_a + o, h_b + o, h_labels + o) != SPKD_OK)
                bad.store(1);
        }
    };
    const int nthreads = (int)std::min<int64_t>(8, n_problems / 16);
    if (nthreads <= 1) {
        work(0, n_problems);
    } else {
        std::vector<std::thread> pool;
        const int64_t step = (n_problems + nthreads - 1) / nthreads;
        for (int t = 0; t < nthreads; ++t) {
            const int64_t lo = t * step, hi = std::min<int64_t>(n_problems, lo + step);
            if (lo < hi) pool.emplace_back(work, lo, hi);
        }
        for (auto& th : pool) th.join();
    }
    return bad.load() ? SPKD_EINVAL : SPKD_OK;
}

}

#ifdef SPKD_PROFILE
extern "C" int spkd_debug_ahc_prof(unsigned long long* out4) {
    unsigned long long z[8] = {0, 0, 0, 0, 0, 0, 0, 0};
    if (hipMemcpyFromSymbol(out4, HIP_SYMBOL(spkd::g_ahc_prof), sizeof z) != hipSuccess) return 1;
    if (hipMemcpyToSymbol(HIP_SYMBOL(spkd::g_ahc_prof), z, sizeof z) != hipSuccess) return 1;
    return 0;
}

extern "C" int spkd_debug_step_prof(unsigned long long* out8) {
    unsigned long long z[8] = {0, 0, 0, 0, 0, 0, 0, 0};
    if (hipMemcpyFromSymbol(out8, HIP_SYMBOL(spkd::g_step_prof), sizeof z) != hipSuccess) return 1;
    if (hipMemcpyToSymbol(HIP_SYMBOL(spkd::g_step_prof), z, sizeof z) != hipSuccess) return 1;
    return 0;
}

extern "C" int spkd_debug_pass_prof(unsigned long long* out4) {
    unsigned long long z[4] = {0, 0, 0, 0};
    if (hipMemcpyFromSymbol(out4, HIP_SYMBOL(spkd::g_pass_prof), sizeof z) != hipSuccess) return 1;
    if (hipMemcpyToSymbol(HIP_SYMBOL(spkd::g_pass_prof), z, sizeof z) != hipSuccess) return 1;
    return 0;
}

extern "C" int spkd_debug_gw_prof(unsigned long long* out12) {
    unsigned long long z[12] = {0, 0, 0, 0, 0, 0, 0, 0, 0, 0, 0, 0};
    if (hipMemcpyFromSymbol(out12, HIP_SYMBOL(spkd::g_gw_prof), sizeof z) != hipSuccess) return 1;
    if (hipMemcpyToSymbol(HIP_SYMBOL(spkd::g_gw_prof), z, sizeof z) != hipSuccess) return 1;
    return 0;
}
#endif
```

### speaker-diarization_amd/hipabi.py

```python
import ctypes as C
import os

import numpy as np

HERE = os.path.dirname(os.path.abspath(__file__))
LIB_PATH = os.environ.get('SPKD_HIP_LIBRARY') or os.path.join(HERE, 'csrc', 'libspkd_hip.so')

SPKD_OK, SPKD_EINVAL, SPKD_EHIP, SPKD_ENONFINITE, SPKD_EOVERFLOW, SPKD_ENOMEM = range(6)
KINDS = {'BIC': 0, 'GLR': 1, 'KL2': 2, 'KL2P': 3}
WANT_GLR, WANT_KL2, WANT_KL2_PINV = 1, 2, 4
TIMERS = {n: i for i, n in enumerate(['call', 'chunk_stats', 'reduce_sets', 'pair_terms',
                                        'cluster_prep', 'matrix', 'ahc', 'gw', 'sw'])}
REC = 820
DIM = 39

EXPORTS = ['spkd_abi_version', 'spkd_create', 'spkd_create_on_stream', 'spkd_destroy', 'spkd_last_error', 'spkd_sync',
           'spkd_malloc', 'spkd_free', 'spkd_memcpy_h2d', 'spkd_memcpy_d2h', 'spkd_memcpy_d2d',
           'spkd_last_kernel_ms', 'spkd_last_gw_items', 'spkd_set_stats', 'spkd_pair_terms',
           'spkd_distance_matrix', 'spkd_gw_event_capacity', 'spkd_gw_event_capacity_p', 'spkd_gw', 'spkd_gw_ex', 'spkd_gw_fused', 'spkd_gather_stats', 'spkd_mfcc',
           'spkd_sw_window_count', 'spkd_sw', 'spkd_ahc', 'spkd_ahc_matrix', 'spkd_distance_rows', 'spkd_cluster_in', 'spkd_py2_roundtrip',
           'spkd_labels_from_merges', 'spkd_labels_from_merges_batch', 'spkd_count_flags', 'spkd_gw_lines',
           'spkd_gmm_loglik', 'spkd_vad_viterbi']


class CdParams(C.Structure):
    _fields_ = [('kind', C.c_int32), ('trace', C.c_int32), ('lambdac', C.c_double),
                ('threshold', C.c_double), ('winsize', C.c_double), ('winstep', C.c_double),
                ('deltaws', C.c_double), ('rate', C.c_double)]


class CandLog(C.Structure):
    _fields_ = [('turn', C.c_int32), ('coarse', C.c_int32), ('seq', C.c_int64),
                ('start', C.c_double), ('i', C.c_double), ('d', C.c_double),
                ('n1', C.c_int64), ('n2', C.c_int64)]


AHC_AUTO, AHC_MONO, AHC_WIDE = 0, 1, 2


class MfccParams(C.Structure):
    _fields_ = [('sample_rate', C.c_int32), ('frame_rate', C.c_int32), ('window_width', C.c_int32),
                ('n_fft', C.c_int32), ('n_mel', C.c_int32), ('n_cep', C.c_int32), ('cms_left', C.c_int32),
                ('cms_right', C.c_int32), ('delta_width', C.c_int32 * 2), ('pre_emph', C.c_float),
                ('delta_norm', C.c_float * 2)]


class GmmParams(C.Structure):
    _fields_ = [('n_kernels', C.c_int32), ('n_states', C.c_int32), ('dim', C.c_int32), ('mean', C.c_void_p),
                ('inv_var', C.c_void_p), ('log_norm', C.c_void_p), ('state_off', C.c_void_p), ('kernel', C.c_void_p),
                ('log_weight', C.c_void_p)]


class AhcParams(C.Structure):
    _fields_ = [('variant', C.c_int32), ('kind', C.c_int32), ('max_spk', C.c_int32),
                ('path', C.c_int32), ('lambdac', C.c_double), ('threshold', C.c_double)]


class SpkdError(RuntimeError):
    def __init__(self, status, text):
        RuntimeError.__init__(self, 'spkd status %d: %s' % (status, text))
        self.status = status


_lib = None


def _one_hip_runtime():
    import sys
    if 'torch' in sys.modules or os.environ.get('SPKD_SYSTEM_HIP'):
        return
    try:
        import importlib.util
        spec = importlib.util.find_spec('torch')
        where = list(spec.submodule_search_locations)[0] if spec and spec.submodule_search_locations else None
    except (ImportError, ValueError, AttributeError):
        where = None
    if where:
        rt = os.path.join(where, 'lib', 'libamdhip64.so')
        if os.path.exists(rt):
            try:
                C.CDLL(rt, mode=C.RTLD_GLOBAL)
            except OSError:
                pass


def mapped_hip_runtimes():
    found = set()
    try:
        with open('/proc/self/maps') as f:
            for line in f:
                path = line.rsplit(None, 1)[-1] if '/' in line else ''
                if os.path.basename(path).startswith('libamdhip64.so'):
                    found.add(os.path.realpath(path))
    except OSError:
        pass
    return sorted(found)


def _check_one_runtime():
    rts = mapped_hip_runtimes()
    if len(rts) > 1:
        raise ImportError('two HIP runtimes are mapped into this process (%s): libspkd_hip.so and the PyTorch '
                          'wheel link against different libamdhip64 sonames.  Set SPKD_SYSTEM_HIP=1 for a '
                          'torch-free process, or import torch before this package.' % ', '.join(rts))


def load_library(path=None):
    global _lib
    if _lib is not None and path is None:
        return _lib
    p = path or LIB_PATH
    if not os.path.exists(p):
        raise ImportError('HIP extension %s is not built: run `python -c "import __graft_entry__ as g; '
                          'g.build()"` (or make -C speaker-diarization_amd/csrc)' % p)
    _one_hip_runtime()
    lib = C.CDLL(p)
    _check_one_runtime()
    vp, i64, i32, dbl = C.c_void_p, C.c_int64, C.c_int32, C.c_double
    P = C.POINTER
    lib.spkd_abi_version.restype = C.c_int
    lib.spkd_create.argtypes = [C.c_int, vp, P(vp)]
    lib.spkd_create_on_stream.argtypes = [C.c_int, vp, P(vp)]
    lib.spkd_destroy.argtypes = [vp]
    lib.spkd_destroy.restype = None
    lib.spkd_last_error.argtypes = [vp]
    lib.spkd_last_error.restype = C.c_char_p
    lib.spkd_sync.argtypes = [vp]
    lib.spkd_malloc.argtypes = [vp, C.c_size_t, P(vp)]
    lib.spkd_free.argtypes = [vp, vp]
    lib.spkd_memcpy_h2d.argtypes = [vp, vp, vp, C.c_size_t]
    lib.spkd_memcpy_d2h.argtypes = [vp, vp, vp, C.c_size_t]
    lib.spkd_memcpy_d2d.argtypes = [vp, vp, vp, C.c_size_t]
    lib.spkd_last_kernel_ms.argtypes = [vp, C.c_int, P(C.c_float)]
    lib.spkd_last_gw_items.argtypes = [vp, P(C.c_int64)]
    lib.spkd_set_stats.argtypes = [vp, vp, i64, vp, vp, vp, i64, i64, vp]
    lib.spkd_pair_terms.argtypes = [vp, vp, vp, vp, i64, C.c_int, vp]
    lib.spkd_distance_matrix.argtypes = [vp, C.c_int, dbl, vp, i64, vp]
    lib.spkd_gw_event_capacity.argtypes = [i64, dbl]
    lib.spkd_gw_event_capacity.restype = i64
    lib.spkd_gw_event_capacity_p.argtypes = [i64, P(CdParams)]
    lib.spkd_gw_event_capacity_p.restype = i64
    lib.spkd_gw.argtypes = [vp, vp, i64, vp, vp, i64, P(CdParams), vp, vp, vp, vp, vp, vp, vp, vp,
                            vp, i64, P(i64)]
    lib.spkd_gw_ex.argtypes = [vp, vp, i64, vp, vp, i64, P(CdParams), vp, C.c_int, vp, vp, vp, vp, vp, vp,
                               vp, vp, i64, P(i64)]
    lib.spkd_gw_fused.argtypes = [vp, vp, i64, vp, vp, i64, P(CdParams), vp, C.c_int, vp, vp, vp, vp, vp, vp,
                                  vp, vp, vp, i64, P(i64)]
    lib.spkd_gather_stats.argtypes = [vp, vp, i64, vp, vp, i64, i64, vp]
    lib.spkd_mfcc.argtypes = [vp, vp, i64, P(MfccParams), vp, vp, vp, vp, vp, vp, P(i64)]
    lib.spkd_sw_window_count.argtypes = [i64, dbl, dbl]
    lib.spkd_sw_window_count.restype = i64
    lib.spkd_sw.argtypes = [vp, vp, i64, vp, vp, i64, P(CdParams), vp, vp]
    lib.spkd_ahc.argtypes = [vp, vp, vp, i64, P(AhcParams), vp, vp, vp, vp, vp, vp]
    lib.spkd_ahc_matrix.argtypes = [vp, vp, i64, P(AhcParams), vp, dbl, dbl, vp, vp, vp, vp, vp, vp]
    lib.spkd_distance_rows.argtypes = [vp, C.c_int, C.c_int, dbl, vp, i64, i64, i64, vp, P(dbl), P(dbl)]
    lib.spkd_cluster_in.argtypes = [vp, vp, i64, C.c_int, dbl, dbl, vp, vp, i64, vp, P(i64), P(i64)]
    lib.spkd_py2_roundtrip.argtypes = [vp, i64]
    lib.spkd_py2_roundtrip.restype = None
    lib.spkd_labels_from_merges.argtypes = [i64, i64, vp, vp, vp]
    lib.spkd_labels_from_merges_batch.argtypes = [i64, vp, vp, vp, vp, vp]
    lib.spkd_count_flags.argtypes = [vp, vp, vp, i64, vp]
    lib.spkd_gmm_loglik.argtypes = [vp, vp, i64, P(GmmParams), vp]
    lib.spkd_vad_viterbi.argtypes = [i64, i32, vp, i32, vp, vp, vp, vp, vp, vp, P(i64), P(dbl)]
    lib.spkd_gw_lines.argtypes = [i64, vp, vp, vp, vp, vp, vp, vp, vp, vp, dbl, C.c_int, i64, vp, vp, vp, vp, vp]
    if lib.spkd_abi_version() != 2:
        raise ImportError('libspkd_hip.so ABI version mismatch')
    if path is None:
        _lib = lib
    return lib


def _ptr(a):
    return a.ctypes.data_as(C.c_void_p)


def py2_roundtrip(values):
    v = np.ascontiguousarray(values, dtype=np.float64).copy()
    if v.size:
        load_library().spkd_py2_roundtrip(_ptr(v), v.size)
    return v


def labels_from_merges(n, a, b):
    a = np.ascontiguousarray(a, dtype=np.int32)
    b = np.ascontiguousarray(b, dtype=np.int32)
    out = np.zeros(n, dtype=np.int32)
    st = load_library().spkd_labels_from_merges(n, len(a), _ptr(a), _ptr(b), _ptr(out))
    if st != SPKD_OK:
        raise SpkdError(st, 'bad merge log')
    return out


def count_flags(flags, off, n):
    flags = np.ascontiguousarray(flags, dtype=np.int32)
    off = np.ascontiguousarray(off, dtype=np.int64)
    n = np.ascontiguousarray(n, dtype=np.int32)
    if len(off) != len(n):
        raise SpkdError(SPKD_EINVAL, 'one offset per group')
    if len(n) and (int((off + n).max()) > len(flags) or int(n.min()) < 0 or int(off.min()) < 0):
        raise SpkdError(SPKD_EINVAL, 'flag ranges outside the array')
    out = np.zeros(len(n), dtype=np.int32)
    st = load_library().spkd_count_flags(_ptr(flags), _ptr(off), _ptr(n), len(n), _ptr(out))
    if st != SPKD_OK:
        raise SpkdError(st, 'bad flag ranges')
    return out


def gw_lines(off, n_det, det_start, det_maxi, final_start, turn_start_s, turn_end_s, turn_begin, turn_end,
             rate, text_contract=True, want_frames=False):
    c = np.ascontiguousarray
    off = c(off, dtype=np.int64); n_det = c(n_det, dtype=np.int32)
    nt = len(n_det)
    arrs = [c(det_start, dtype=np.float64), c(det_maxi, dtype=np.float64), c(final_start, dtype=np.float64),
            c(turn_start_s, dtype=np.float64), c(turn_end_s, dtype=np.float64), c(turn_begin, dtype=np.int64),
            c(turn_end, dtype=np.int64)]
    if len(off) != nt or any(len(a) != nt for a in arrs[2:]):
        raise SpkdError(SPKD_EINVAL, 'one entry per turn')
    if nt and (int(n_det.min()) < 0 or int(off.min()) < 0 or int((off + n_det).max()) > min(len(arrs[0]), len(arrs[1]))):
        raise SpkdError(SPKD_EINVAL, 'detections outside the event arrays')
    n_lines = int(n_det.sum(dtype=np.int64)) + nt
    times = np.empty((n_lines, 2), dtype=np.float64)
    turn = np.empty(n_lines, dtype=np.int32)
    fb = np.empty(n_lines, dtype=np.int64) if want_frames else None
    fe = np.empty(n_lines, dtype=np.int64) if want_frames else None
    ix = np.empty(n_lines, dtype=np.int64) if want_frames else None
    p = lambda a: _ptr(a) if a is not None else None
    st = load_library().spkd_gw_lines(nt, _ptr(off), _ptr(n_det), *[_ptr(a) for a in arrs], float(rate),
                                      1 if text_contract else 0, n_lines, _ptr(times), p(fb), p(fe), p(ix), _ptr(turn))
    if st != SPKD_OK:
        raise SpkdError(st, 'bad growing-window result')
    return {'times': times, 'turn': turn, 'frame_b': fb, 'frame_e': fe, 'index': ix}


def vad_viterbi(scores, word_state, stay, exit_, enter):
    c = np.ascontiguousarray
    scores = c(scores, dtype=np.float32)
    if scores.ndim != 2:
        raise SpkdError(SPKD_EINVAL, 'scores must be [frames, states]')
    ws = c(word_state, dtype=np.int32)
    consts = [c(a, dtype=np.float64) for a in (stay, exit_, enter)]
    if any(len(a) != len(ws) for a in consts):
        raise SpkdError(SPKD_EINVAL, 'one constant of each kind per word')
    T, S = scores.shape
    tf = np.zeros(max(T, 1), dtype=np.int64)
    tw = np.zeros(max(T, 1), dtype=np.int32)
    n = C.c_int64(0)
    sc = C.c_double(0.0)
    st = load_library().spkd_vad_viterbi(T, S, _ptr(scores), len(ws), _ptr(ws), *[_ptr(a) for a in consts],
                                         _ptr(tf), _ptr(tw), C.byref(n), C.byref(sc))
    if st != SPKD_OK:
        raise SpkdError(st, 'bad decoder input')
    return tf[:n.value].copy(), tw[:n.value].copy(), sc.value


def labels_from_merges_batch(seg_off, n_merges, a, b):
    seg_off = np.ascontiguousarray(seg_off, dtype=np.int64)
    n_merges = np.ascontiguousarray(n_merges, dtype=np.int32)
    a = np.ascontiguousarray(a, dtype=np.int32)
    b = np.ascontiguousarray(b, dtype=np.int32)
    out = np.zeros(int(seg_off[-1]), dtype=np.int32)
    st = load_library().spkd_labels_from_merges_batch(len(seg_off) - 1, _ptr(seg_off), _ptr(n_merges),
                                                      _ptr(a), _ptr(b), _ptr(out))
    if st != SPKD_OK:
        raise SpkdError(st, 'bad merge log')
    return out


class Context(object):

    def __init__(self, device=0, stream=None):
        self.lib = load_library()
        h = C.c_void_p()
        if stream is None:
            st = self.lib.spkd_create(int(device), None, C.byref(h))
        else:
            st = self.lib.spkd_create_on_stream(int(device), C.c_void_p(int(stream)), C.byref(h))
        if st != SPKD_OK:
            raise SpkdError(st, 'spkd_create failed (no usable HIP device %d?)' % device)
        self.h = h
        self.device = device

    def close(self):
        if getattr(self, 'h', None):
            for ptr, _ in self.__dict__.pop('_dev_scratch', {}).values():
                self.lib.spkd_free(self.h, C.c_void_p(ptr))
            self.lib.spkd_destroy(self.h)
            self.h = None

    def __del__(self):
        try:
            self.close()
        except Exception:
            pass

    def check(self, st, allow=()):
        if st != SPKD_OK and st not in allow:
            raise SpkdError(st, self.lib.spkd_last_error(self.h).decode())
        return st

    def last_ms(self, which='call'):
        ms = C.c_float()
        self.check(self.lib.spkd_last_kernel_ms(self.h, TIMERS[which], C.byref(ms)))
        return ms.value

    def last_gw_items(self):
        n = C.c_int64()
        self.check(self.lib.spkd_last_gw_items(self.h, C.byref(n)))
        return int(n.value)

    def dev_alloc(self, nbytes):
        p = C.c_void_p()
        self.check(self.lib.spkd_malloc(self.h, nbytes, C.byref(p)))
        return p.value

    def dev_free(self, ptr):
        if ptr:
            self.check(self.lib.spkd_free(self.h, C.c_void_p(ptr)))

    def dev_scratch(self, name, nbytes):
        cache = self.__dict__.setdefault('_dev_scratch', {})
        ptr, cap = cache.get(name, (None, 0))
        if ptr is None or cap < nbytes:
            if ptr is not None:
                self.dev_free(ptr)
            ptr, cap = self.dev_alloc(nbytes), nbytes
            cache[name] = (ptr, cap)
        return ptr

    def h2d(self, dptr, arr):
        arr = np.ascontiguousarray(arr)
        self.check(self.lib.spkd_memcpy_h2d(self.h, C.c_void_p(dptr), _ptr(arr), arr.nbytes))

    def copy_d2d(self, d_dst, d_src, nbytes):
        self.check(self.lib.spkd_memcpy_d2d(self.h, C.c_void_p(d_dst), C.c_void_p(d_src), int(nbytes)))

    def d2h(self, arr, dptr):
        assert arr.flags['C_CONTIGUOUS']
        self.check(self.lib.spkd_memcpy_d2h(self.h, _ptr(arr), C.c_void_p(dptr), arr.nbytes))

    def set_stats(self, d_frames, n_frames, begins, ends, sets, n_sets, d_stats):
        b = np.ascontiguousarray(begins, dtype=np.int64)
        e = np.ascontiguousarray(ends, dtype=np.int64)
        s = np.ascontiguousarray(sets, dtype=np.int32)
        self.check(self.lib.spkd_set_stats(self.h, C.c_void_p(d_frames), n_frames, _ptr(b), _ptr(e),
                                           _ptr(s), len(b), n_sets, C.c_void_p(d_stats)))

    def pair_terms(self, d_stats, ia, ib, flags=0):
        ia = np.ascontiguousarray(ia, dtype=np.int32)
        ib = np.ascontiguousarray(ib, dtype=np.int32)
        out = np.empty((len(ia), 8), dtype=np.float64)
        st = self.lib.spkd_pair_terms(self.h, C.c_void_p(d_stats), _ptr(ia), _ptr(ib), len(ia),
                                      flags, _ptr(out))
        self.check(st, allow=(SPKD_ENONFINITE,))
        return out, st

    def distance_matrix(self, kind, lambdac, d_stats, n, d_matrix):
        st = self.lib.spkd_distance_matrix(self.h, KINDS[kind], lambdac, C.c_void_p(d_stats), n,
                                           C.c_void_p(d_matrix))
        return self.check(st, allow=(SPKD_ENONFINITE,))

    def _buf(self, name, n, dtype):
        cache = self.__dict__.setdefault('_bufs', {})
        arr = cache.get(name)
        if arr is None or arr.shape[0] < n or arr.dtype != np.dtype(dtype):
            arr = cache[name] = np.empty(max(n, 1), dtype=dtype)
        return arr[:n]

    def gather_stats(self, d_src, n_src, src_index, d_dst, n_dst, dst_index=None):
        si = np.ascontiguousarray(src_index, dtype=np.int64)
        di = None if dst_index is None else np.ascontiguousarray(dst_index, dtype=np.int64)
        self.check(self.lib.spkd_gather_stats(self.h, C.c_void_p(d_src), n_src, _ptr(si),
                                              None if di is None else _ptr(di), len(si), n_dst,
                                              C.c_void_p(d_dst)))

    def gw(self, d_frames, n_frames, begins, ends, params, log_cap=4096, tight=False, reuse=False,
           seg_stats=None, first_guess_scale=1.0):
        b = np.ascontiguousarray(begins, dtype=np.int64)
        e = np.ascontiguousarray(ends, dtype=np.int64)
        nt = len(b)
        if not (params.rate >= 10.0 and params.winstep >= 1.0):
            raise SpkdError(SPKD_EINVAL, 'unsupported growing-window parameters (frame rate >= 10 and '
                                         'a window step of at least one frame needed)')
        step = min(0.2 * params.rate, 0.5 * params.rate, params.winstep)
        full = ((e - b).astype(np.float64) / step).astype(np.int64) + 8
        if first_guess_scale != 1.0:
            full = np.maximum((full * float(first_guess_scale)).astype(np.int64), 2)
        grow = 1
        while True:
            caps = (full // 4 + 8) if tight else full * grow
            off = np.zeros(nt + 1, dtype=np.int64)
            off[1:] = np.cumsum(caps)
            nev = int(off[-1])
            mk = self._buf if reuse else (lambda name, n, dt: np.empty(n, dtype=dt))
            n_win = mk('n_win', nt, np.int32)
            win_maxd = mk('win_maxd', nev, np.float64)
            win_det = mk('win_det', nev, np.int32)
            det_start = mk('det_start', nev, np.float64)
            det_maxi = mk('det_maxi', nev, np.float64)
            det_d = mk('det_d', nev, np.float64)
            final_start = mk('final_start', nt, np.float64)
            log = (CandLog * max(log_cap, 1))()
            cnt = C.c_int64(0)
            if seg_stats is None:
                st = self.lib.spkd_gw_ex(self.h, C.c_void_p(d_frames), n_frames, _ptr(b), _ptr(e), nt,
                                         C.byref(params), _ptr(off), 0, _ptr(n_win),
                                         _ptr(win_maxd), _ptr(win_det), _ptr(det_start), _ptr(det_maxi),
                                         _ptr(det_d), _ptr(final_start), C.cast(log, C.c_void_p), log_cap,
                                         C.byref(cnt))
            else:
                d_seg = seg_stats(nev)
                st = self.lib.spkd_gw_fused(self.h, C.c_void_p(d_frames), n_frames, _ptr(b), _ptr(e), nt,
                                            C.byref(params), _ptr(off), 0, _ptr(n_win),
                                            _ptr(win_maxd), _ptr(win_det), _ptr(det_start), _ptr(det_maxi),
                                            _ptr(det_d), _ptr(final_start), C.c_void_p(d_seg),
                                            C.cast(log, C.c_void_p), log_cap, C.byref(cnt))
            if st == SPKD_EOVERFLOW and cnt.value > log_cap:
                log_cap = int(cnt.value) + 16
                continue
            if st == SPKD_EOVERFLOW and tight:
                tight = False
                continue
            if st == SPKD_EOVERFLOW and grow < 1024:
                grow *= 2
                continue
            self.check(st, allow=(SPKD_ENONFINITE,))
            break
        return dict(status=st, off=off, n_ev=nev, n_win=n_win, win_maxd=win_maxd, win_det=win_det,
                    det_start=det_start, det_maxi=det_maxi, det_d=det_d, final_start=final_start,
                    log=log, log_count=min(int(cnt.value), log_cap))

    def sw(self, d_frames, n_frames, begins, ends, params):
        b = np.ascontiguousarray(begins, dtype=np.int64)
        e = np.ascontiguousarray(ends, dtype=np.int64)
        nt = len(b)
        cnt = [self.lib.spkd_sw_window_count(int(e[t] - b[t]), params.winsize, params.winstep)
               for t in range(nt)]
        if any(c < 0 for c in cnt):
            raise SpkdError(SPKD_EINVAL, 'window size and step must be at least one frame')
        off = np.zeros(nt + 1, dtype=np.int64)
        off[1:] = np.cumsum(cnt)
        d = np.zeros(int(off[-1]), dtype=np.float64)
        st = self.lib.spkd_sw(self.h, C.c_void_p(d_frames), n_frames, _ptr(b), _ptr(e), nt,
                              C.byref(params), _ptr(off), _ptr(d))
        self.check(st, allow=(SPKD_ENONFINITE,))
        return st, off, d

    def mfcc(self, d_pcm, n_samples, params, melfb, dct, mean, scale, transform, d_features):
        arrs = [np.ascontiguousarray(a, dtype=np.float32) for a in (melfb, dct, mean, scale, transform)]
        n = C.c_int64(0)
        self.check(self.lib.spkd_mfcc(self.h, C.c_void_p(d_pcm), n_samples, C.byref(params), *[_ptr(a) for a in arrs],
                                      C.c_void_p(d_features), C.byref(n)))
        return int(n.value)

    def gmm_loglik(self, d_features, n_frames, gmm, d_scores):
        a = {k: np.ascontiguousarray(gmm[k], dtype=np.int32 if k in ('state_off', 'kernel') else np.float32)
             for k in ('mean', 'inv_var', 'log_norm', 'state_off', 'kernel', 'log_weight')}
        K, S = len(a['log_norm']), len(a['state_off']) - 1
        if a['mean'].size != K * DIM or a['inv_var'].size != K * DIM or S < 1 or \
                len(a['kernel']) != len(a['log_weight']) or int(a['state_off'][-1]) != len(a['kernel']):
            raise SpkdError(SPKD_EINVAL, 'inconsistent model array sizes')
        p = GmmParams(K, S, a['mean'].shape[-1] if a['mean'].ndim == 2 else DIM,
                      *[_ptr(a[k]) for k in ('mean', 'inv_var', 'log_norm', 'state_off', 'kernel', 'log_weight')])
        self.check(self.lib.spkd_gmm_loglik(self.h, C.c_void_p(d_features), int(n_frames), C.byref(p),
                                            C.c_void_p(d_scores)))

    def ahc(self, d_stats, seg_off, params):
        seg_off = np.ascontiguousarray(seg_off, dtype=np.int64)
        npb = len(seg_off) - 1
        nt = int(seg_off[-1])
        n_merges = np.zeros(npb, dtype=np.int32)
        ma = np.zeros(nt, dtype=np.int32)
        mb = np.zeros(nt, dtype=np.int32)
        md = np.zeros(nt, dtype=np.float64)
        smax = np.zeros(npb, dtype=np.float64)
        smin = np.zeros(npb, dtype=np.float64)
        st = self.lib.spkd_ahc(self.h, C.c_void_p(d_stats), _ptr(seg_off), npb, C.byref(params),
                               _ptr(n_merges), _ptr(ma), _ptr(mb), _ptr(md), _ptr(smax), _ptr(smin))
        self.check(st, allow=(SPKD_ENONFINITE,))
        return dict(status=st, n_merges=n_merges, a=ma, b=mb, d=md, stat_max=smax, stat_min=smin)

    def distance_rows(self, variant, kind, lambdac, d_stats, n, row_begin, row_end, d_rows):
        smax, smin = C.c_double(), C.c_double()
        st = self.lib.spkd_distance_rows(self.h, int(variant), KINDS[kind] if isinstance(kind, str) else int(kind),
                                         float(lambdac), C.c_void_p(d_stats), int(n), int(row_begin), int(row_end),
                                         C.c_void_p(d_rows), C.byref(smax), C.byref(smin))
        self.check(st, allow=(SPKD_ENONFINITE,))
        if st == SPKD_ENONFINITE:
            raise ValueError('array must not contain infs or NaNs')
        return smax.value, smin.value

    def cluster_in(self, d_stats, n, kind, lambdac, threshold):
        n = int(n)
        label = np.zeros(max(n, 1), dtype=np.int32)
        off = np.zeros(n + 1, dtype=np.int64)
        done, nclu = C.c_int64(0), C.c_int64(0)
        full = n * (n - 1) // 2
        cap = min(full, 32 * n)
        while True:
            dist = np.empty(max(cap, 1), dtype=np.float64)
            st = self.lib.spkd_cluster_in(self.h, C.c_void_p(d_stats), n, KINDS[kind] if isinstance(kind, str) else int(kind),
                                          float(lambdac), float(threshold), _ptr(label), _ptr(dist), cap, _ptr(off),
                                          C.byref(done), C.byref(nclu))
            if st == SPKD_EOVERFLOW and cap < full:
                cap = min(full, 4 * cap)
                continue
            break
        self.check(st, allow=(SPKD_ENONFINITE,))
        nd = int(done.value)
        dists = [dist[int(off[s]):int(off[s + 1])].copy() for s in range(nd)]
        return label[:n], dists, nd, int(nclu.value), st

    def ahc_matrix(self, d_stats, n, params, d_matrix, stat_max_in=float('nan'), stat_min_in=float('nan')):
        n = int(n)
        n_merges = np.zeros(1, dtype=np.int32)
        ma = np.zeros(n, dtype=np.int32)
        mb = np.zeros(n, dtype=np.int32)
        md = np.zeros(n, dtype=np.float64)
        smax = np.zeros(1, dtype=np.float64)
        smin = np.zeros(1, dtype=np.float64)
        st = self.lib.spkd_ahc_matrix(self.h, C.c_void_p(d_stats), n, C.byref(params), C.c_void_p(d_matrix),
                                      float(stat_max_in), float(stat_min_in), _ptr(n_merges), _ptr(ma), _ptr(mb),
                                      _ptr(md), _ptr(smax), _ptr(smin))
        self.check(st, allow=(SPKD_ENONFINITE,))
        return dict(status=st, n_merges=n_merges, a=ma, b=mb, d=md, stat_max=smax, stat_min=smin)
```

### speaker-diarization_amd/pipeline.py

```python
import time

import numpy as np

from . import hipabi
from .recipe import py2_float_str

DIA2_CD = dict(kind='BIC', lambdac=1.0, threshold=0.0, winsize_s=1.0, winstep_s=3.0, deltaws_s=0.1)
DIA2_CL = dict(variant=1, kind='BIC', lambdac=1.3, threshold=0.0, max_spk=0)


class BatchFile(object):

    def __init__(self, frame_off, n_frames, vad):
        self.frame_off = int(frame_off)
        self.n_frames = int(n_frames)
        self.vad = [(float(s), float(e)) for (s, e) in vad]
        self.vad_arr = np.array(self.vad, dtype=np.float64).reshape(-1, 2)


class FusedStats(object):

    def __init__(self, d_buf, n_buf, index, begin, end):
        self.d_buf, self.n_buf, self.index, self.begin, self.end = d_buf, n_buf, index, begin, end


def change_detect_batch(ctx, d_frames, total_frames, files, rate=125.0, cd=DIA2_CD, timings=None,
                        text_contract=True, fused=None):
    rate = float(rate)
    _t0 = time.perf_counter()
    nturn = [len(f.vad) for f in files]
    if sum(nturn) == 0:
        return [[] for _ in files]
    vad = np.concatenate([f.vad_arr for f in files])
    owner = np.repeat(np.arange(len(files)), nturn)
    foff = np.array([f.frame_off for f in files], dtype=np.int64)[owner]
    fn = np.array([f.n_frames for f in files], dtype=np.int64)[owner]
    ls, le = vad[:, 0], vad[:, 1]
    f0 = np.minimum((ls * rate).astype(np.int64), fn)
    f1 = np.maximum(f0, np.minimum((le * rate).astype(np.int64), fn))
    tb, te = foff + f0, foff + f1
    p = hipabi.CdParams(hipabi.KINDS[cd['kind']], 0, cd['lambdac'], cd['threshold'],
                        float(np.floor(cd['winsize_s'] * rate)), float(np.floor(cd['winstep_s'] * rate)),
                        float(np.floor(rate * cd['deltaws_s'])), rate)
    _t1 = time.perf_counter()
    seg_buf = {}

    def seg_alloc(n_rec):
        seg_buf['n'] = n_rec
        seg_buf['p'] = ctx.dev_scratch('fused_segment_stats', max(n_rec, 1) * hipabi.REC * 8)
        return seg_buf['p']

    r = ctx.gw(d_frames, total_frames, tb, te, p, log_cap=4096, tight=True, reuse=True,
               seg_stats=seg_alloc if fused is not None else None)
    _t2 = time.perf_counter()
    if timings is not None:
        timings.setdefault('gw', []).append(ctx.last_ms('gw'))
        timings.setdefault('gw_stream_ms', []).append(ctx.last_ms('call'))
        timings['gw_frames'] = int((te - tb).sum())
        timings['gw_windows'] = int(r['n_win'].sum())
        timings['gw_dets'] = ctx.last_gw_items()
    if r['status'] == hipabi.SPKD_ENONFINITE:
        raise ValueError('array must not contain infs or NaNs')
    off = r['off']
    nt = len(tb)
    nd = hipabi.count_flags(r['win_det'], off[:-1], r['n_win'])
    lines = hipabi.gw_lines(off[:-1], nd, r['det_start'], r['det_maxi'], r['final_start'], ls, le, tb, te, rate,
                            text_contract=text_contract, want_frames=fused is not None)
    rt, line_turn = lines['times'], lines['turn']
    if fused is not None:
        fused.append(FusedStats(seg_buf['p'], seg_buf['n'], lines['index'], lines['frame_b'], lines['frame_e']))
    line_file = owner[line_turn]
    bounds = np.searchsorted(line_file, np.arange(len(files) + 1))
    out = [rt[bounds[i]:bounds[i + 1]] for i in range(len(files))]
    if timings is not None:
        _t3 = time.perf_counter()
        timings.setdefault('wall_cd_prepare', []).append(1e3 * (_t1 - _t0))
        timings.setdefault('wall_cd_call', []).append(1e3 * (_t2 - _t1))
        timings.setdefault('wall_cd_finish', []).append(1e3 * (_t3 - _t2))
    return out


def segment_stats(ctx, d_frames, total_frames, files, segments, rate=125.0, timings=None, fused=None,
                  scratch_name='segment_stats'):
    cnt = [len(s) for s in segments]
    seg_off = np.zeros(len(files) + 1, dtype=np.int64)
    seg_off[1:] = np.cumsum(cnt)
    n = int(seg_off[-1])
    allseg = np.concatenate([np.asarray(s, dtype=np.float64).reshape(-1, 2) for s in segments]) if n else np.zeros((0, 2))
    owner = np.repeat(np.arange(len(files)), cnt)
    foff = np.array([f.frame_off for f in files], dtype=np.int64)[owner]
    fn = np.array([f.n_frames for f in files], dtype=np.int64)[owner]
    a0 = np.clip((allseg[:, 0] * rate).astype(np.int64), 0, fn)
    a1 = np.maximum(a0, np.clip((allseg[:, 1] * rate).astype(np.int64), 0, fn))
    b, e = foff + a0, foff + a1
    d_stats = ctx.dev_scratch(scratch_name, max(n, 1) * hipabi.REC * 8)
    _t1 = time.perf_counter()
    if fused is None:
        ctx.set_stats(d_frames, total_frames, b, e, np.arange(n, dtype=np.int32), n, d_stats)
        redo = np.arange(n)
    else:
        same = (fused.begin == b) & (fused.end == e)
        keep = np.nonzero(same)[0]
        redo = np.nonzero(~same)[0]
        ctx.gather_stats(fused.d_buf, fused.n_buf, fused.index[keep], d_stats, n, keep)
        if len(redo):
            d_tmp = ctx.dev_scratch(scratch_name + '_redo', len(redo) * hipabi.REC * 8)
            ctx.set_stats(d_frames, total_frames, b[redo], e[redo], np.arange(len(redo), dtype=np.int32),
                          len(redo), d_tmp)
            ctx.gather_stats(d_tmp, len(redo), np.arange(len(redo)), d_stats, n, redo)
    if timings is not None:
        if len(redo):
            timings.setdefault('chunk_stats', []).append(ctx.last_ms('chunk_stats'))
            timings.setdefault('reduce_sets', []).append(ctx.last_ms('reduce_sets'))
        timings['stats_frames'] = int((e[redo] - b[redo]).sum())
        timings['stats_sets'] = n
        timings['stats_recomputed'] = int(len(redo))
    return d_stats, seg_off, n, _t1


def cluster_batch(ctx, d_frames, total_frames, files, segments, rate=125.0, cl=DIA2_CL, timings=None,
                  want_merges=False, fused=None):
    rate = float(rate)
    if fused is None and any(len(sg) == 0 for sg in segments):
        keep = [i for i, sg in enumerate(segments) if len(sg) > 0]
        out = [(np.zeros(0, dtype=np.int32), [] if want_merges else None) for _ in files]
        if keep:
            sub = cluster_batch(ctx, d_frames, total_frames, [files[i] for i in keep],
                                [segments[i] for i in keep], rate, cl, timings, want_merges)
            for i, r in zip(keep, sub):
                out[i] = r
        return out
    _t0 = time.perf_counter()
    cnt = [len(s) for s in segments]
    d_stats, seg_off, n, _t1 = segment_stats(ctx, d_frames, total_frames, files, segments, rate, timings, fused)
    _t2 = time.perf_counter()
    p = hipabi.AhcParams(cl['variant'], hipabi.KINDS[cl['kind']], cl['max_spk'], cl.get('path', 0),
                         cl['lambdac'], cl['threshold'])
    r = ctx.ahc(d_stats, seg_off, p)
    _t3 = time.perf_counter()
    if timings is not None:
        for k in ('cluster_prep', 'matrix', 'ahc'):
            timings.setdefault(k, []).append(ctx.last_ms(k))
        npb = np.diff(seg_off)
        nm = r['n_merges'].astype(np.int64)
        timings['matrix_pairs'] = int((npb * (npb - 1) // 2).sum())
        timings['ahc_pairs'] = int((nm * (npb - 2) - nm * (nm - 1) // 2).sum())
    if r['status'] == hipabi.SPKD_ENONFINITE:
        raise ValueError('array must not contain infs or NaNs')
    all_labels = hipabi.labels_from_merges_batch(seg_off, r['n_merges'], r['a'], r['b'])
    out = []
    for fi in range(len(files)):
        o, c = int(seg_off[fi]), cnt[fi]
        merges = None
        if want_merges:
            nm = int(r['n_merges'][fi])
            merges = list(zip(r['a'][o:o + nm].tolist(), r['b'][o:o + nm].tolist(), r['d'][o:o + nm].tolist()))
        out.append((all_labels[o:o + c], merges))
    if timings is not None:
        _t4 = time.perf_counter()
        timings.setdefault('wall_cl_prepare', []).append(1e3 * (_t1 - _t0))
        timings.setdefault('wall_cl_stats_call', []).append(1e3 * (_t2 - _t1))
        timings.setdefault('wall_cl_ahc_call', []).append(1e3 * (_t3 - _t2))
        timings.setdefault('wall_cl_finish', []).append(1e3 * (_t4 - _t3))
    return out


def diarize_batch(ctx, d_frames, total_frames, files, rate=125.0, cd=DIA2_CD, cl=DIA2_CL, timings=None,
                  text_contract=True, fused=False):
    box = [] if fused else None
    segs = change_detect_batch(ctx, d_frames, total_frames, files, rate, cd, timings, text_contract, box)
    fs = box[0] if box else None
    if fused and fs is None:
        return [np.zeros((0, 3)) for _ in files]
    if fused and any(len(sg) == 0 for sg in segs):
        keep = [i for i, sg in enumerate(segs) if len(sg) > 0]
        out = [np.zeros((0, 3)) for _ in files]
        if keep:
            sub = _cluster_and_order(ctx, d_frames, total_frames, [files[i] for i in keep],
                                     [segs[i] for i in keep], rate, cl, timings, fs)
            for i, rws in zip(keep, sub):
                out[i] = rws
        return out
    return _cluster_and_order(ctx, d_frames, total_frames, files, segs, rate, cl, timings, fs)


def _cluster_and_order(ctx, d_frames, total_frames, files, segs, rate, cl, timings, fs):
    res = cluster_batch(ctx, d_frames, total_frames, files, segs, rate, cl, timings, fused=fs)
    cnt = [len(s) for s in segs]
    n = sum(cnt)
    if n == 0:
        return [np.zeros((0, 3)) for _ in segs]
    allseg = np.concatenate([np.asarray(s, dtype=np.float64).reshape(-1, 2) for s in segs])
    labels = np.concatenate([lab for (lab, _) in res]).astype(np.float64)
    owner = np.repeat(np.arange(len(segs)), cnt)
    k0, k1 = allseg[:, 0] * rate, allseg[:, 1] * rate
    in_order = (owner[1:] != owner[:-1]) | (k0[1:] > k0[:-1]) | ((k0[1:] == k0[:-1]) & (k1[1:] >= k1[:-1]))
    if bool(in_order.all()):
        rows = np.column_stack([allseg, labels])
    else:
        order = np.lexsort((np.arange(n), k1, k0, owner))
        rows = np.column_stack([allseg[order], labels[order]])
    bounds = np.zeros(len(segs) + 1, dtype=np.int64)
    bounds[1:] = np.cumsum(cnt)
    out = [rows[bounds[i]:bounds[i + 1]] for i in range(len(segs))]
    return out


def in_flight(contexts, n_jobs, job):
    import threading
    if len(contexts) == 1 or n_jobs <= 1:
        for k in range(n_jobs):
            yield job(contexts[0], k)
        return
    results = [None] * n_jobs
    done = [threading.Event() for _ in range(n_jobs)]
    nxt = [0]
    lock = threading.Lock()
    failure = []

    def worker(ctx):
        while not failure:
            with lock:
                k = nxt[0]
                nxt[0] += 1
            if k >= n_jobs:
                return
            try:
                results[k] = job(ctx, k)
            except BaseException as e:
                failure.append(e)
            finally:
                done[k].set()

    threads = [threading.Thread(target=worker, args=(c,)) for c in contexts]
    for th in threads:
        th.start()
    try:
        for k in range(n_jobs):
            done[k].wait()
            if failure:
                break
            r, results[k] = results[k], None
            yield r
    finally:
        if not failure:
            failure.append(None)
        for th in threads:
            th.join()
    if failure and failure[0] is not None:
        raise failure[0]
```

Before: 1411.

## Keep change-detection-to-clustering handoff on device with GPU line compaction

Adds a device-side handoff path. Detected segments are compacted into lines on the GPU with count, scan and emit kernels and copied back through pinned buffers. Clustering then gathers per-segment stats on device through an index map, recomputing only the segments that need it. This removes the host round trips, the Python-side segment assembly and the separate stats gather call between change detection and AHC. In exchange it adds several new kernels, a single-block scan, and a new API surface whose correctness depends on the redo-map patching.

Result: faster. 1447, median of 6 (+2.6%).

```diff
diff --git a/include/spkd.h b/include/spkd.h
--- a/include/spkd.h
+++ b/include/spkd.h
@@ -121,6 +121,28 @@
                               const int64_t *h_src_index, const int64_t *h_dst_index,
                               int64_t n, int64_t n_dst, double *d_dst);
 
+typedef struct {
+    int64_t n_lines;
+    int64_t n_redo;
+    const int32_t *n_win;
+    const double *times;
+    const int32_t *turn;
+    const int64_t *frame_b;
+    const int64_t *frame_e;
+    const int64_t *index;
+    const int64_t *d_index;
+    const int64_t *redo_line;
+    const int64_t *redo_begin;
+    const int64_t *redo_end;
+} spkd_gw_lines_view;
+
+spkd_status spkd_gw_batch(spkd_ctx *ctx, const float *d_frames, int64_t n_frames,
+                          const int64_t *h_turn_begin, const int64_t *h_turn_end, int64_t n_turns,
+                          const spkd_cd_params *params, const int64_t *h_ev_off,
+                          const double *h_turn_start_s, const double *h_turn_end_s,
+                          const int64_t *h_turn_file_off, const int64_t *h_turn_file_len,
+                          double *d_seg_stats, int want_index, spkd_gw_lines_view *view);
+
 int64_t spkd_sw_window_count(int64_t turn_len, double winsize, double winstep);
 spkd_status spkd_sw(spkd_ctx *ctx, const float *d_frames, int64_t n_frames,
                     const int64_t *h_turn_begin, const int64_t *h_turn_end, int64_t n_turns,
@@ -146,6 +168,16 @@
                             const double *d_matrix, double stat_max_in, double stat_min_in,
                             int32_t *h_n_merges, int32_t *h_merge_a, int32_t *h_merge_b,
                             double *h_merge_d, double *h_stat_max, double *h_stat_min);
+
+spkd_status spkd_ahc_fused(spkd_ctx *ctx, const float *d_frames, int64_t n_frames,
+                           const double *d_records, int64_t n_records, int64_t *d_line_index,
+                           const int64_t *h_seg_off, int64_t n_problems,
+                           const int64_t *h_redo_line, const int64_t *h_redo_begin,
+                           const int64_t *h_redo_end, int64_t n_redo,
+                           const spkd_ahc_params *params,
+                           const int32_t **h_n_merges, const int32_t **h_merge_a,
+                           const int32_t **h_merge_b, const double **h_merge_d,
+                           const int32_t **h_labels);
 
 typedef struct {
     int32_t sample_rate, frame_rate, window_width, n_fft, n_mel, n_cep;
diff --git a/speaker-diarization_amd/csrc/spkd_hip.hip b/speaker-diarization_amd/csrc/spkd_hip.hip
--- a/speaker-diarization_amd/csrc/spkd_hip.hip
+++ b/speaker-diarization_amd/csrc/spkd_hip.hip
@@ -21,7 +21,8 @@
 using namespace spkd;
 
 namespace {
-constexpr int N_SLOTS = 36;
+constexpr int N_SLOTS = 40;
+enum { PIN_GW_TURNS = 0, PIN_GW_LINES, PIN_AHC_OUT, N_PIN };
 }
 
 struct spkd_ctx {
@@ -46,6 +47,12 @@
     size_t slot_bytes[N_SLOTS] = {};
     void* pinv_ws = nullptr;
     double* pinv_cur = nullptr;
+    void* pin[N_PIN] = {};
+    size_t pin_bytes[N_PIN] = {};
+    std::vector<int64_t> redo_line, redo_begin, redo_end;
+    std::vector<Chunk> redo_chunks;
+    std::vector<int64_t> redo_setoff;
+    std::vector<int32_t> redo_sets;
 };
 
 namespace {
@@ -80,6 +87,23 @@
         c->slot_bytes[slot] = want;
     }
     *out = c->slot[slot];
+    return SPKD_OK;
+}
+
+spkd_status pinned(spkd_ctx* c, int which, size_t bytes, void** out) {
+    if (bytes == 0) bytes = 16;
+    if (c->pin_bytes[which] < bytes) {
+        if (c->pin[which]) HIPCHK(c, hipHostFree(c->pin[which]));
+        c->pin[which] = nullptr;
+        c->pin_bytes[which] = 0;
+        const size_t want = bytes + bytes / 4;
+        if (hipHostMalloc(&c->pin[which], want, hipHostMallocDefault) != hipSuccess) {
+            c->pin[which] = nullptr;
+            return fail(c, SPKD_ENOMEM, "pinned host allocation failed");
+        }
+        c->pin_bytes[which] = want;
+    }
+    *out = c->pin[which];
     return SPKD_OK;
 }
 
@@ -151,7 +175,8 @@
     S_CHUNKS = 0, S_SETOFF, S_PARTIAL, S_IDXA, S_IDXB, S_TERMS, S_TURNS, S_SNAP, S_CAND,
     S_EV_I32A, S_EV_I32B, S_EV_D0, S_EV_D1, S_EV_D2, S_EV_D3, S_EV_D4, S_LOG,
     S_AHC_STATS, S_AHC_LD, S_AHC_AUX, S_AHC_MAT, S_AHC_MISC, S_AHC_OUT, S_AHC_OFF, S_AHC_PROB, S_AHC_PACKED, S_MFCC_TAB, S_MFCC_STATIC,
-    S_STEP_EXM, S_STEP_PKM, S_STEP_MISC, S_GMM_TAB, S_GMM_IDX, S_COUNT
+    S_STEP_EXM, S_STEP_PKM, S_STEP_MISC, S_GMM_TAB, S_GMM_IDX,
+    S_CP_TURNS, S_CP_TIMES, S_CP_LINES, S_REDO_STATS, S_REDO_IDX, S_COUNT
 };
 static_assert(S_COUNT <= N_SLOTS, "scratch slot table too small");
 
@@ -216,6 +241,8 @@
         if (c->slot[i]) (void)hipFree(c->slot[i]);
     if (c->d_err) (void)hipFree(c->d_err);
     if (c->pinv_ws) (void)hipFree(c->pinv_ws);
+    for (int i = 0; i < N_PIN; ++i)
+        if (c->pin[i]) (void)hipHostFree(c->pin[i]);
     if (c->d_counter) (void)hipFree(c->d_counter);
     if (c->ev0) (void)hipEventDestroy(c->ev0);
     if (c->ev1) (void)hipEventDestroy(c->ev1);
@@ -390,7 +417,53 @@
     const double* d_init = nullptr;
     double init_max = NAN, init_min = NAN;
     int64_t row_begin = -1, row_end = -1;
+    int64_t* d_map = nullptr;
+    int64_t n_src = 0;
+    const float* d_frames = nullptr;
+    int64_t n_frames = 0;
+    const int64_t *redo_line = nullptr, *redo_begin = nullptr, *redo_end = nullptr;
+    int64_t n_redo = 0;
 };
+
+__global__ __launch_bounds__(256) void k_patch_map(const int64_t* __restrict__ line, int64_t n, int64_t* __restrict__ map) {
+    const int64_t k = (int64_t)blockIdx.x * 256 + threadIdx.x;
+    if (k < n) map[line[k]] = -(k + 1);
+}
+
+__global__ __launch_bounds__(256) void k_records_from_map(const double* __restrict__ recs, int64_t n_recs,
+                                                          const int64_t* __restrict__ map,
+                                                          const double* __restrict__ redo, int64_t n_redo,
+                                                          int64_t n_rec, double* __restrict__ qr,
+                                                          double* __restrict__ packed, int* __restrict__ err) {
+    const int64_t c = blockIdx.x;
+    if (c >= n_rec) return;
+    const int64_t m = map[c];
+    const double* g;
+    if (m >= 0 && m < n_recs) {
+        g = recs + m * REC;
+    } else if (m < 0 && -(m + 1) < n_redo) {
+        g = redo + (-(m + 1)) * REC;
+    } else {
+        if (threadIdx.x == 0) atomicOr(err, 4);
+        return;
+    }
+    double* o = qr + c * QREC;
+    for (int e = threadIdx.x; e < QREC; e += 256) {
+        const int t = e & 15, sj = e >> 4;
+        const int s = sj / DA, j = sj - s * DA;
+        double v = 0.0;
+        if (t < QL) {
+            const int i = QL * s + t;
+            const int r = i < j ? i : j, cc = i < j ? j : i;
+            v = g[pk(r, cc)];
+        } else if (e == QREC_COUNT_AT) {
+            v = g[REC - 1];
+        }
+        o[e] = v;
+    }
+    double* p = packed + c * REC;
+    for (int e = threadIdx.x; e < REC; e += 256) p[e] = g[e];
+}
 
 spkd_status ahc_prepare(spkd_ctx* c, const double* d_stats, const int64_t* h_seg_off, int64_t n_prob,
                         int variant, int kind, double lambdac, AhcBuffers& B, int64_t& n_total,
@@ -469,8 +542,25 @@
     TRY(scratch(c, S_AHC_PACKED, (size_t)n_total * REC * sizeof(double), &p));
     B.pk = (double*)p;
     if (n_total > 0) {
-        hipLaunchKernelGGL(k_to_quadrec, dim3((unsigned)n_total), dim3(256), 0, c->stream, d_stats, n_total, B.ex);
-        HIPCHK(c, hipMemcpyAsync(B.pk, d_stats, (size_t)n_total * REC * sizeof(double), hipMemcpyDeviceToDevice, c->stream));
+        if (plan.d_map) {
+            void* d_redo = nullptr;
+            if (plan.n_redo > 0) {
+                int64_t* d_rl = nullptr;
+                TRY(scratch(c, S_REDO_STATS, (size_t)plan.n_redo * REC * sizeof(double), &d_redo));
+                TRY(upload(c, S_REDO_IDX, plan.redo_line, (size_t)plan.n_redo, &d_rl));
+                c->redo_sets.resize((size_t)plan.n_redo);
+                for (int64_t k = 0; k < plan.n_redo; ++k) c->redo_sets[(size_t)k] = (int32_t)k;
+                TRY(set_stats_launch(c, plan.d_frames, plan.n_frames, plan.redo_begin, plan.redo_end, c->redo_sets.data(),
+                                     plan.n_redo, plan.n_redo, (double*)d_redo, c->redo_chunks, c->redo_setoff));
+                hipLaunchKernelGGL(k_patch_map, dim3((unsigned)((plan.n_redo + 255) / 256)), dim3(256), 0, c->stream,
+                                   (const int64_t*)d_rl, plan.n_redo, plan.d_map);
+            }
+            hipLaunchKernelGGL(k_records_from_map, dim3((unsigned)n_total), dim3(256), 0, c->stream, d_stats, plan.n_src,
+                               (const int64_t*)plan.d_map, (const double*)d_redo, plan.n_redo, n_total, B.ex, B.pk, c->d_err);
+        } else {
+            hipLaunchKernelGGL(k_to_quadrec, dim3((unsigned)n_total), dim3(256), 0, c->stream, d_stats, n_total, B.ex);
+            HIPCHK(c, hipMemcpyAsync(B.pk, d_stats, (size_t)n_total * REC * sizeof(double), hipMemcpyDeviceToDevice, c->stream));
+        }
         const int64_t per_block = kind == SPKD_KL2 ? PT_WAVES : 4 * PT_WAVES;
         const unsigned blocks = (unsigned)((n_total + per_block - 1) / per_block);
         {
@@ -826,18 +916,222 @@
 }
 
 namespace {
+constexpr int CP_TPB = 256;
+constexpr int CP_SCAN_TPB = 1024;
+
+__global__ __launch_bounds__(CP_TPB) void k_cp_count(const TurnDesc* __restrict__ turns, int64_t n_turns,
+                                                     const int32_t* __restrict__ n_win,
+                                                     const int32_t* __restrict__ win_det, const int* __restrict__ err,
+                                                     int32_t* __restrict__ n_det, int32_t* __restrict__ pos) {
+    if (*err) return;
+    const int64_t p = (int64_t)blockIdx.x * CP_TPB + threadIdx.x;
+    if (p >= n_turns) return;
+    const TurnDesc T = turns[p];
+    int64_t nw = n_win[T.id];
+    nw = nw < 0 ? 0 : (nw > T.ev_cap ? T.ev_cap : nw);
+    const int32_t* f = win_det + T.ev_off;
+    int32_t cnt = 0;
+    for (int64_t i = 0; i < nw; ++i) cnt += f[i] != 0;
+    n_det[T.id] = cnt;
+    pos[T.id] = (int32_t)p;
+}
+
+__global__ __launch_bounds__(CP_SCAN_TPB) void k_cp_scan(const int32_t* __restrict__ n_det, int64_t n_turns,
+                                                         const int* __restrict__ err, int64_t* __restrict__ line_off) {
+    __shared__ int64_t part[CP_SCAN_TPB];
+    const int tid = threadIdx.x;
+    if (*err) {
+        if (tid == 0) line_off[n_turns] = 0;
+        return;
+    }
+    const int64_t per = (n_turns + CP_SCAN_TPB - 1) / CP_SCAN_TPB;
+    const int64_t lo = tid * per < n_turns ? tid * per : n_turns;
+    const int64_t hi = lo + per < n_turns ? lo + per : n_turns;
+    int64_t sum = 0;
+    for (int64_t t = lo; t < hi; ++t) sum += (int64_t)n_det[t] + 1;
+    part[tid] = sum;
+    __syncthreads();
+    for (int d = 1; d < CP_SCAN_TPB; d <<= 1) {
+        const int64_t v = tid >= d ? part[tid - d] : 0;
+        __syncthreads();
+        part[tid] += v;
+        __syncthreads();
+    }
+    int64_t run = part[tid] - sum;
+    for (int64_t t = lo; t < hi; ++t) {
+        line_off[t] = run;
+        run += (int64_t)n_det[t] + 1;
+    }
+    if (tid == CP_SCAN_TPB - 1) line_off[n_turns] = part[tid];
+}
+
+__global__ __launch_bounds__(CP_TPB) void k_cp_lines(const TurnDesc* __restrict__ turns, int64_t n_turns,
+                                                     const int32_t* __restrict__ n_det, const int32_t* __restrict__ pos,
+                                                     const int64_t* __restrict__ line_off, int64_t n_lines,
+                                                     const double* __restrict__ det_start,
+                                                     const double* __restrict__ det_maxi,
+                                                     const double* __restrict__ final_start,
+                                                     const double* __restrict__ turn_start_s,
+                                                     const double* __restrict__ turn_end_s, double rate,
+                                                     const int* __restrict__ err, double* __restrict__ times,
+                                                     int64_t* __restrict__ frame_b, int64_t* __restrict__ frame_e,
+                                                     int64_t* __restrict__ index, int32_t* __restrict__ line_turn) {
+#pragma clang fp contract(off)
+    if (*err) return;
+    const int64_t t = (int64_t)blockIdx.x * CP_TPB + threadIdx.x;
+    if (t >= n_turns) return;
+    const TurnDesc T = turns[pos[t]];
+    const int64_t nd = n_det[t];
+    const double ls = turn_start_s[t], le = turn_end_s[t];
+    int64_t i = line_off[t];
+    for (int64_t j = 0; j <= nd && i < n_lines; ++j, ++i) {
+        const bool tail = j == nd;
+        double fs, fe;
+        if (tail) {
+            fs = final_start[t];
+            times[2 * i] = fs / rate + ls;
+            times[2 * i + 1] = ((le - ls) * rate) / rate + ls;
+            fe = 0.0;
+        } else {
+            fs = det_start[T.ev_off + j];
+            fe = fs + det_maxi[T.ev_off + j];
+            times[2 * i] = fs / rate + ls;
+            times[2 * i + 1] = fe / rate + ls;
+        }
+        frame_b[i] = T.begin + (int64_t)fs;
+        frame_e[i] = tail ? T.begin + T.len : T.begin + (int64_t)fe;
+        index[i] = T.ev_off + j;
+        line_turn[i] = (int32_t)t;
+    }
+}
+
+struct GwBatch {
+    const double *turn_start_s, *turn_end_s;
+    const int64_t *file_off, *file_len;
+    int want_index;
+    spkd_gw_lines_view* view;
+    double *d_ls = nullptr, *d_le = nullptr;
+    int64_t* d_line_off = nullptr;
+    int32_t *d_n_det = nullptr, *d_pos = nullptr;
+    int64_t* h_head = nullptr;
+    int32_t* h_n_win = nullptr;
+    int64_t n_lines = 0;
+    bool have_lines = false;
+};
+
+spkd_status gw_batch_upload(spkd_ctx* c, GwBatch& G, int64_t n_turns) {
+    const size_t nt = (size_t)n_turns;
+    void *p = nullptr, *h = nullptr;
+    TRY(scratch(c, S_CP_TURNS, nt * (2 * sizeof(double) + 2 * sizeof(int32_t)) + (nt + 1) * sizeof(int64_t), &p));
+    G.d_ls = (double*)p;
+    G.d_le = G.d_ls + nt;
+    G.d_line_off = (int64_t*)(G.d_le + nt);
+    G.d_n_det = (int32_t*)(G.d_line_off + nt + 1);
+    G.d_pos = G.d_n_det + nt;
+    HIPCHK(c, hipMemcpyAsync(G.d_ls, G.turn_start_s, nt * sizeof(double), hipMemcpyHostToDevice, c->stream));
+    HIPCHK(c, hipMemcpyAsync(G.d_le, G.turn_end_s, nt * sizeof(double), hipMemcpyHostToDevice, c->stream));
+    TRY(pinned(c, PIN_GW_TURNS, 2 * sizeof(int64_t) + nt * sizeof(int32_t), &h));
+    G.h_head = (int64_t*)h;
+    G.h_n_win = (int32_t*)(G.h_head + 2);
+    return SPKD_OK;
+}
+
+spkd_status gw_batch_compact(spkd_ctx* c, GwBatch& G, const TurnDesc* d_turns, int64_t n_turns,
+                             const int32_t* d_n_win, const int32_t* d_win_det, const double* d_det_start,
+                             const double* d_det_maxi, const double* d_final_start, double rate) {
+    const unsigned blocks = (unsigned)((n_turns + CP_TPB - 1) / CP_TPB);
+    hipLaunchKernelGGL(k_cp_count, dim3(blocks), dim3(CP_TPB), 0, c->stream, d_turns, n_turns, d_n_win, d_win_det,
+                       (const int*)c->d_err, G.d_n_det, G.d_pos);
+    hipLaunchKernelGGL(k_cp_scan, dim3(1), dim3(CP_SCAN_TPB), 0, c->stream, (const int32_t*)G.d_n_det, n_turns,
+                       (const int*)c->d_err, G.d_line_off);
+    HIPCHK(c, hipGetLastError());
+    G.h_head[0] = 0;
+    G.h_head[1] = 0;
+    HIPCHK(c, hipMemcpyAsync(&G.h_head[0], G.d_line_off + n_turns, sizeof(int64_t), hipMemcpyDeviceToHost, c->stream));
+    HIPCHK(c, hipMemcpyAsync(&G.h_head[1], c->d_err, sizeof(int), hipMemcpyDeviceToHost, c->stream));
+    HIPCHK(c, hipMemcpyAsync(G.h_n_win, d_n_win, (size_t)n_turns * sizeof(int32_t), hipMemcpyDeviceToHost, c->stream));
+    HIPCHK(c, hipStreamSynchronize(c->stream));
+    if (G.h_head[1] != 0) return SPKD_OK;
+    const int64_t n = G.h_head[0];
+    if (n < n_turns) return fail(c, SPKD_EHIP, "internal error: fewer lines than turns");
+    const size_t nn = (size_t)n;
+    void *d_t = nullptr, *d_l = nullptr, *h = nullptr;
+    TRY(scratch(c, S_CP_TIMES, nn * 2 * sizeof(double), &d_t));
+    TRY(scratch(c, S_CP_LINES, nn * (3 * sizeof(int64_t) + sizeof(int32_t)), &d_l));
+    TRY(pinned(c, PIN_GW_LINES, nn * (2 * sizeof(double) + 3 * sizeof(int64_t) + sizeof(int32_t)), &h));
+    int64_t* d_fb = (int64_t*)d_l;
+    int64_t* d_ix = d_fb + 2 * nn;
+    int32_t* d_tn = (int32_t*)(d_ix + nn);
+    hipLaunchKernelGGL(k_cp_lines, dim3(blocks), dim3(CP_TPB), 0, c->stream, d_turns, n_turns,
+                       (const int32_t*)G.d_n_det, (const int32_t*)G.d_pos, (const int64_t*)G.d_line_off, n, d_det_start,
+                       d_det_maxi, d_final_start, (const double*)G.d_ls, (const double*)G.d_le, rate,
+                       (const int*)c->d_err, (double*)d_t, d_fb, d_fb + nn, d_ix, d_tn);
+    HIPCHK(c, hipGetLastError());
+    double* h_times = (double*)h;
+    int64_t* h_fb = (int64_t*)(h_times + 2 * nn);
+    int64_t* h_ix = h_fb + 2 * nn;
+    int32_t* h_tn = (int32_t*)(h_ix + nn);
+    HIPCHK(c, hipMemcpyAsync(h_times, d_t, nn * 2 * sizeof(double), hipMemcpyDeviceToHost, c->stream));
+    HIPCHK(c, hipMemcpyAsync(h_fb, d_fb, nn * 2 * sizeof(int64_t), hipMemcpyDeviceToHost, c->stream));
+    HIPCHK(c, hipMemcpyAsync(h_tn, d_tn, nn * sizeof(int32_t), hipMemcpyDeviceToHost, c->stream));
+    if (G.want_index)
+        HIPCHK(c, hipMemcpyAsync(h_ix, d_ix, nn * sizeof(int64_t), hipMemcpyDeviceToHost, c->stream));
+    spkd_gw_lines_view& V = *G.view;
+    V.n_lines = n;
+    V.n_win = G.h_n_win;
+    V.times = h_times;
+    V.turn = h_tn;
+    V.frame_b = h_fb;
+    V.frame_e = h_fb + nn;
+    V.index = G.want_index ? h_ix : nullptr;
+    V.d_index = d_ix;
+    G.n_lines = n;
+    G.have_lines = true;
+    return SPKD_OK;
+}
+
+spkd_status gw_batch_finish(spkd_ctx* c, GwBatch& G, int64_t n_turns, double rate) {
+    spkd_gw_lines_view& V = *G.view;
+    double* times = const_cast<double*>(V.times);
+    spkd_py2_roundtrip(times, 2 * V.n_lines);
+    c->redo_line.clear();
+    c->redo_begin.clear();
+    c->redo_end.clear();
+    for (int64_t i = 0; i < V.n_lines; ++i) {
+        const int64_t t = V.turn[i];
+        if (t < 0 || t >= n_turns) return fail(c, SPKD_EHIP, "internal error: line of no turn");
+        const int64_t fn = G.file_len[t];
+        int64_t a0 = (int64_t)(times[2 * i] * rate), a1 = (int64_t)(times[2 * i + 1] * rate);
+        a0 = a0 < 0 ? 0 : (a0 > fn ? fn : a0);
+        a1 = a1 < 0 ? 0 : (a1 > fn ? fn : a1);
+        if (a1 < a0) a1 = a0;
+        const int64_t b = G.file_off[t] + a0, e = G.file_off[t] + a1;
+        if (b != V.frame_b[i] || e != V.frame_e[i]) {
+            c->redo_line.push_back(i);
+            c->redo_begin.push_back(b);
+            c->redo_end.push_back(e);
+        }
+    }
+    V.n_redo = (int64_t)c->redo_line.size();
+    V.redo_line = c->redo_line.data();
+    V.redo_begin = c->redo_begin.data();
+    V.redo_end = c->redo_end.data();
+    return SPKD_OK;
+}
+
 constexpr int64_t GW_WAVE_PER_TURN_FROM = 4096;
 constexpr int64_t GW_EIGHT_WAVES_UP_TO = 256;
 spkd_status gw_impl(spkd_ctx* c, const float* d_frames, int64_t n_frames, const int64_t* hb,
                     const int64_t* he, int64_t n_turns, const spkd_cd_params* P, const int64_t* h_ev_off,
                     int check_capacity, int32_t* h_n_win, double* h_win_maxd, int32_t* h_win_det,
                     double* h_det_start, double* h_det_maxi, double* h_det_d, double* h_final_start,
-                    double* d_seg_stats, spkd_cand_log* h_log, int64_t log_cap, int64_t* h_log_count) {
+                    double* d_seg_stats, spkd_cand_log* h_log, int64_t log_cap, int64_t* h_log_count,
+                    GwBatch* batch = nullptr) {
     if (!c || !P || n_turns < 0) return SPKD_EINVAL;
     if (h_log_count) *h_log_count = 0;
     if (n_turns == 0) return SPKD_OK;
-    if (!d_frames || !hb || !he || !h_ev_off || !h_n_win || !h_win_maxd || !h_win_det || !h_det_start ||
-        !h_det_maxi || !h_det_d || !h_final_start)
+    if (!d_frames || !hb || !he || !h_ev_off) return fail(c, SPKD_EINVAL, "null argument");
+    if (!batch && (!h_n_win || !h_win_maxd || !h_win_det || !h_det_start || !h_det_maxi || !h_det_d || !h_final_start))
         return fail(c, SPKD_EINVAL, "null argument");
     if (P->kind < 0 || P->kind > 3) return fail(c, SPKD_EINVAL, "gw: bad kind");
     if (!(P->rate >= 10.0) || !(P->winsize >= 1.0) || !(P->winstep >= 1.0))
@@ -875,6 +1169,7 @@
         !d_log || !c->d_counter || !c->d_err)
         return fail(c, SPKD_EHIP, "gw: a device scratch buffer is missing");
     HIPCHK(c, hipMemsetAsync(c->d_counter, 0, 2 * sizeof(unsigned long long), c->stream));
+    if (batch) TRY(gw_batch_upload(c, *batch, n_turns));
     int nw = c->gw_waves;
     if (nw != 1 && nw != 2 && nw != 4 && nw != 8)
         nw = n_turns >= GW_WAVE_PER_TURN_FROM ? 1 : (n_turns <= GW_EIGHT_WAVES_UP_TO ? 8 : 4);
@@ -892,6 +1187,16 @@
 #undef SPKD_GW_LAUNCH
     HIPCHK(c, hipGetLastError());
     unsigned long long& cnt = cnt2[0];
+    if (batch) {
+        TRY(gw_batch_compact(c, *batch, d_turns, n_turns, (const int32_t*)d_i32a, (const int32_t*)d_i32b,
+                             (const double*)d_d1, (const double*)d_d2, (const double*)d_d4, P->rate));
+        HIPCHK(c, hipMemcpyAsync(cnt2, c->d_counter, sizeof cnt2, hipMemcpyDeviceToHost, c->stream));
+        const spkd_status st = call.finish();
+        c->last_gw_items = (int64_t)cnt2[1];
+        if (st != SPKD_OK) return st;
+        if (!batch->have_lines) return fail(c, SPKD_EHIP, "internal error: no lines from a clean call");
+        return gw_batch_finish(c, *batch, n_turns, P->rate);
+    }
     HIPCHK(c, hipMemcpyAsync(h_n_win, d_i32a, (size_t)n_turns * sizeof(int32_t), hipMemcpyDeviceToHost, c->stream));
     HIPCHK(c, hipMemcpyAsync(h_win_maxd, d_d0, (size_t)n_ev * sizeof(double), hipMemcpyDeviceToHost, c->stream));
     HIPCHK(c, hipMemcpyAsync(h_win_det, d_i32b, (size_t)n_ev * sizeof(int32_t), hipMemcpyDeviceToHost, c->stream));
@@ -941,6 +1246,81 @@
     return gw_impl(c, d_frames, n_frames, hb, he, n_turns, P, h_ev_off, check_capacity, h_n_win, h_win_maxd,
                    h_win_det, h_det_start, h_det_maxi, h_det_d, h_final_start, d_seg_stats, h_log, log_cap,
                    h_log_count);
+}
+
+spkd_status spkd_gw_batch(spkd_ctx* c, const float* d_frames, int64_t n_frames, const int64_t* hb,
+                          const int64_t* he, int64_t n_turns, const spkd_cd_params* P, const int64_t* h_ev_off,
+                          const double* h_turn_start_s, const double* h_turn_end_s, const int64_t* h_turn_file_off,
+                          const int64_t* h_turn_file_len, double* d_seg_stats, int want_index,
+                          spkd_gw_lines_view* view) {
+    if (!c || !view) return SPKD_EINVAL;
+    std::memset(view, 0, sizeof *view);
+    if (!d_seg_stats) return fail(c, SPKD_EINVAL, "gw_batch: null statistics buffer");
+    if (n_turns > 0 && (!h_turn_start_s || !h_turn_end_s || !h_turn_file_off || !h_turn_file_len))
+        return fail(c, SPKD_EINVAL, "gw_batch: null turn arrays");
+    GwBatch G;
+    G.turn_start_s = h_turn_start_s;
+    G.turn_end_s = h_turn_end_s;
+    G.file_off = h_turn_file_off;
+    G.file_len = h_turn_file_len;
+    G.want_index = want_index;
+    G.view = view;
+    const spkd_status st = gw_impl(c, d_frames, n_frames, hb, he, n_turns, P, h_ev_off, 0, nullptr, nullptr, nullptr,
+                                   nullptr, nullptr, nullptr, nullptr, d_seg_stats, nullptr, 0, nullptr, &G);
+    if (st != SPKD_OK) std::memset(view, 0, sizeof *view);
+    return st;
+}
+
+spkd_status spkd_ahc_fused(spkd_ctx* c, const float* d_frames, int64_t n_frames, const double* d_records,
+                           int64_t n_records, int64_t* d_line_index, const int64_t* h_seg_off, int64_t n_prob,
+                           const int64_t* h_redo_line, const int64_t* h_redo_begin, const int64_t* h_redo_end,
+                           int64_t n_redo, const spkd_ahc_params* P, const int32_t** h_n_merges,
+                           const int32_t** h_merge_a, const int32_t** h_merge_b, const double** h_merge_d,
+                           const int32_t** h_labels) {
+    if (!c || !P || n_prob < 0 || n_redo < 0) return SPKD_EINVAL;
+    if (!h_n_merges || !h_merge_a || !h_merge_b || !h_merge_d || !h_labels)
+        return fail(c, SPKD_EINVAL, "ahc_fused: null output");
+    *h_n_merges = *h_merge_a = *h_merge_b = *h_labels = nullptr;
+    *h_merge_d = nullptr;
+    if (n_prob == 0) return SPKD_OK;
+    if (!d_records || !d_line_index || !h_seg_off || n_records < 1 || h_seg_off[0] != 0)
+        return fail(c, SPKD_EINVAL, "ahc_fused: null argument or first offset not 0");
+    for (int64_t p = 0; p < n_prob; ++p)
+        if (h_seg_off[p + 1] < h_seg_off[p]) return fail(c, SPKD_EINVAL, "seg_off must be non-decreasing");
+    const int64_t n_total = h_seg_off[n_prob];
+    if (n_redo > 0 && (!h_redo_line || !h_redo_begin || !h_redo_end || !d_frames))
+        return fail(c, SPKD_EINVAL, "ahc_fused: null redo arrays");
+    for (int64_t k = 0; k < n_redo; ++k)
+        if (h_redo_line[k] < 0 || h_redo_line[k] >= n_total || (k > 0 && h_redo_line[k] <= h_redo_line[k - 1]))
+            return fail(c, SPKD_EINVAL, "ahc_fused: redo lines must be ascending line indices");
+    const size_t nt = (size_t)n_total, np = (size_t)n_prob;
+    void* h = nullptr;
+    TRY(pinned(c, PIN_AHC_OUT, (nt + 2 * np) * sizeof(double) + (3 * nt + np) * sizeof(int32_t), &h));
+    double* md = (double*)h;
+    double* smax = md + nt;
+    double* smin = smax + np;
+    int32_t* ma = (int32_t*)(smin + np);
+    int32_t* mb = ma + nt;
+    int32_t* lab = mb + nt;
+    int32_t* nm = lab + nt;
+    MatrixPlan plan;
+    plan.d_map = d_line_index;
+    plan.n_src = n_records;
+    plan.d_frames = d_frames;
+    plan.n_frames = n_frames;
+    plan.redo_line = h_redo_line;
+    plan.redo_begin = h_redo_begin;
+    plan.redo_end = h_redo_end;
+    plan.n_redo = n_redo;
+    TRY(ahc_impl(c, d_records, h_seg_off, n_prob, P, plan, nm, ma, mb, md, smax, smin));
+    if (spkd_labels_from_merges_batch(n_prob, h_seg_off, nm, ma, mb, lab) != SPKD_OK)
+        return fail(c, SPKD_EHIP, "internal error: merge log does not replay");
+    *h_n_merges = nm;
+    *h_merge_a = ma;
+    *h_merge_b = mb;
+    *h_merge_d = md;
+    *h_labels = lab;
+    return SPKD_OK;
 }
 
 namespace {
diff --git a/speaker-diarization_amd/hipabi.py b/speaker-diarization_amd/hipabi.py
--- a/speaker-diarization_amd/hipabi.py
+++ b/speaker-diarization_amd/hipabi.py
@@ -17,7 +17,7 @@
 EXPORTS = ['spkd_abi_version', 'spkd_create', 'spkd_create_on_stream', 'spkd_destroy', 'spkd_last_error', 'spkd_sync',
            'spkd_malloc', 'spkd_free', 'spkd_memcpy_h2d', 'spkd_memcpy_d2h', 'spkd_memcpy_d2d',
            'spkd_last_kernel_ms', 'spkd_last_gw_items', 'spkd_set_stats', 'spkd_pair_terms',
-           'spkd_distance_matrix', 'spkd_gw_event_capacity', 'spkd_gw_event_capacity_p', 'spkd_gw', 'spkd_gw_ex', 'spkd_gw_fused', 'spkd_gather_stats', 'spkd_mfcc',
+           'spkd_distance_matrix', 'spkd_gw_event_capacity', 'spkd_gw_event_capacity_p', 'spkd_gw', 'spkd_gw_ex', 'spkd_gw_fused', 'spkd_gw_batch', 'spkd_ahc_fused', 'spkd_gather_stats', 'spkd_mfcc',
            'spkd_sw_window_count', 'spkd_sw', 'spkd_ahc', 'spkd_ahc_matrix', 'spkd_distance_rows', 'spkd_cluster_in', 'spkd_py2_roundtrip',
            'spkd_labels_from_merges', 'spkd_labels_from_merges_batch', 'spkd_count_flags', 'spkd_gw_lines',
            'spkd_gmm_loglik', 'spkd_vad_viterbi']
@@ -33,6 +33,13 @@
     _fields_ = [('turn', C.c_int32), ('coarse', C.c_int32), ('seq', C.c_int64),
                 ('start', C.c_double), ('i', C.c_double), ('d', C.c_double),
                 ('n1', C.c_int64), ('n2', C.c_int64)]
+
+
+class GwLinesView(C.Structure):
+    _fields_ = [('n_lines', C.c_int64), ('n_redo', C.c_int64), ('n_win', C.c_void_p), ('times', C.c_void_p),
+                ('turn', C.c_void_p), ('frame_b', C.c_void_p), ('frame_e', C.c_void_p), ('index', C.c_void_p),
+                ('d_index', C.c_void_p), ('redo_line', C.c_void_p), ('redo_begin', C.c_void_p),
+                ('redo_end', C.c_void_p)]
 
 
 AHC_AUTO, AHC_MONO, AHC_WIDE = 0, 1, 2
@@ -146,6 +153,9 @@
                                vp, vp, i64, P(i64)]
     lib.spkd_gw_fused.argtypes = [vp, vp, i64, vp, vp, i64, P(CdParams), vp, C.c_int, vp, vp, vp, vp, vp, vp,
                                   vp, vp, vp, i64, P(i64)]
+    lib.spkd_gw_batch.argtypes = [vp, vp, i64, vp, vp, i64, P(CdParams), vp, vp, vp, vp, vp, vp, C.c_int, P(GwLinesView)]
+    lib.spkd_ahc_fused.argtypes = [vp, vp, i64, vp, i64, vp, vp, i64, vp, vp, vp, i64, P(AhcParams),
+                                   P(vp), P(vp), P(vp), P(vp), P(vp)]
     lib.spkd_gather_stats.argtypes = [vp, vp, i64, vp, vp, i64, i64, vp]
     lib.spkd_mfcc.argtypes = [vp, vp, i64, P(MfccParams), vp, vp, vp, vp, vp, vp, P(i64)]
     lib.spkd_sw_window_count.argtypes = [i64, dbl, dbl]
@@ -172,6 +182,13 @@
 
 def _ptr(a):
     return a.ctypes.data_as(C.c_void_p)
+
+
+def _view(addr, n, dtype):
+    if not addr or n <= 0:
+        return np.zeros(0, dtype=dtype)
+    ct = {np.int32: C.c_int32, np.int64: C.c_int64, np.float64: C.c_double}[dtype]
+    return np.ctypeslib.as_array(C.cast(C.c_void_p(addr), C.POINTER(ct)), shape=(int(n),))
 
 
 def py2_roundtrip(values):
@@ -429,6 +446,69 @@
                     det_start=det_start, det_maxi=det_maxi, det_d=det_d, final_start=final_start,
                     log=log, log_count=min(int(cnt.value), log_cap))
 
+    def gw_batch(self, d_frames, n_frames, begins, ends, params, turn_start_s, turn_end_s, file_off, file_len,
+                 seg_stats, tight=True, first_guess_scale=1.0, want_index=False):
+        c = np.ascontiguousarray
+        b = c(begins, dtype=np.int64)
+        e = c(ends, dtype=np.int64)
+        nt = len(b)
+        host = [c(turn_start_s, dtype=np.float64), c(turn_end_s, dtype=np.float64), c(file_off, dtype=np.int64),
+                c(file_len, dtype=np.int64)]
+        if any(len(a) != nt for a in host):
+            raise SpkdError(SPKD_EINVAL, 'one entry per turn')
+        if not (params.rate >= 10.0 and params.winstep >= 1.0):
+            raise SpkdError(SPKD_EINVAL, 'unsupported growing-window parameters (frame rate >= 10 and '
+                                         'a window step of at least one frame needed)')
+        step = min(0.2 * params.rate, 0.5 * params.rate, params.winstep)
+        full = ((e - b).astype(np.float64) / step).astype(np.int64) + 8
+        if first_guess_scale != 1.0:
+            full = np.maximum((full * float(first_guess_scale)).astype(np.int64), 2)
+        grow = 1
+        view = GwLinesView()
+        while True:
+            caps = (full // 4 + 8) if tight else full * grow
+            off = np.zeros(nt + 1, dtype=np.int64)
+            off[1:] = np.cumsum(caps)
+            nev = int(off[-1])
+            d_seg = seg_stats(nev)
+            st = self.lib.spkd_gw_batch(self.h, C.c_void_p(d_frames), n_frames, _ptr(b), _ptr(e), nt, C.byref(params),
+                                        _ptr(off), *[_ptr(a) for a in host], C.c_void_p(d_seg),
+                                        1 if want_index else 0, C.byref(view))
+            if st == SPKD_EOVERFLOW and tight:
+                tight = False
+                continue
+            if st == SPKD_EOVERFLOW and grow < 1024:
+                grow *= 2
+                continue
+            self.check(st, allow=(SPKD_ENONFINITE,))
+            break
+        n, nr = int(view.n_lines), int(view.n_redo)
+        return dict(status=st, off=off, n_ev=nev, d_seg=d_seg, n_lines=n, n_win=_view(view.n_win, nt if n else 0, np.int32),
+                    times=_view(view.times, 2 * n, np.float64).reshape(-1, 2), turn=_view(view.turn, n, np.int32),
+                    frame_b=_view(view.frame_b, n, np.int64), frame_e=_view(view.frame_e, n, np.int64),
+                    index=_view(view.index, n, np.int64) if want_index else None, d_index=view.d_index,
+                    redo_line=_view(view.redo_line, nr, np.int64), redo_begin=_view(view.redo_begin, nr, np.int64),
+                    redo_end=_view(view.redo_end, nr, np.int64))
+
+    def ahc_fused(self, d_frames, n_frames, d_records, n_records, d_line_index, seg_off, redo_line, redo_begin,
+                  redo_end, params):
+        c = np.ascontiguousarray
+        seg_off = c(seg_off, dtype=np.int64)
+        rl, rb, re_ = c(redo_line, dtype=np.int64), c(redo_begin, dtype=np.int64), c(redo_end, dtype=np.int64)
+        if not (len(rl) == len(rb) == len(re_)):
+            raise SpkdError(SPKD_EINVAL, 'one range per redo line')
+        npb, nt = len(seg_off) - 1, int(seg_off[-1])
+        out = [C.c_void_p() for _ in range(5)]
+        st = self.lib.spkd_ahc_fused(self.h, C.c_void_p(d_frames), n_frames, C.c_void_p(d_records), n_records,
+                                     C.c_void_p(d_line_index), _ptr(seg_off), npb, _ptr(rl), _ptr(rb), _ptr(re_), len(rl),
+                                     C.byref(params), *[C.byref(o) for o in out])
+        self.check(st, allow=(SPKD_ENONFINITE,))
+        if st != SPKD_OK:
+            return dict(status=st)
+        return dict(status=st, n_merges=_view(out[0].value, npb, np.int32), a=_view(out[1].value, nt, np.int32),
+                    b=_view(out[2].value, nt, np.int32), d=_view(out[3].value, nt, np.float64),
+                    labels=_view(out[4].value, nt, np.int32))
+
     def sw(self, d_frames, n_frames, begins, ends, params):
         b = np.ascontiguousarray(begins, dtype=np.int64)
         e = np.ascontiguousarray(ends, dtype=np.int64)
diff --git a/speaker-diarization_amd/pipeline.py b/speaker-diarization_amd/pipeline.py
--- a/speaker-diarization_amd/pipeline.py
+++ b/speaker-diarization_amd/pipeline.py
@@ -165,8 +165,101 @@
     return out
 
 
+def diarize_batch_device(ctx, d_frames, total_frames, files, rate=125.0, cd=DIA2_CD, cl=DIA2_CL, timings=None,
+                         detail=None, first_guess_scale=1.0):
+    rate = float(rate)
+    _t0 = time.perf_counter()
+    nturn = [len(f.vad) for f in files]
+    if sum(nturn) == 0:
+        return [np.zeros((0, 3)) for _ in files]
+    vad = np.concatenate([f.vad_arr for f in files])
+    owner = np.repeat(np.arange(len(files)), nturn)
+    foff = np.array([f.frame_off for f in files], dtype=np.int64)[owner]
+    fn = np.array([f.n_frames for f in files], dtype=np.int64)[owner]
+    ls, le = np.ascontiguousarray(vad[:, 0]), np.ascontiguousarray(vad[:, 1])
+    f0 = np.minimum((ls * rate).astype(np.int64), fn)
+    f1 = np.maximum(f0, np.minimum((le * rate).astype(np.int64), fn))
+    tb, te = foff + f0, foff + f1
+    p = hipabi.CdParams(hipabi.KINDS[cd['kind']], 0, cd['lambdac'], cd['threshold'],
+                        float(np.floor(cd['winsize_s'] * rate)), float(np.floor(cd['winstep_s'] * rate)),
+                        float(np.floor(rate * cd['deltaws_s'])), rate)
+    _t1 = time.perf_counter()
+    r = ctx.gw_batch(d_frames, total_frames, tb, te, p, ls, le, foff, fn,
+                     lambda n_rec: ctx.dev_scratch('fused_segment_stats', max(n_rec, 1) * hipabi.REC * 8),
+                     tight=True, first_guess_scale=first_guess_scale, want_index=detail is not None)
+    _t2 = time.perf_counter()
+    if timings is not None:
+        timings.setdefault('gw', []).append(ctx.last_ms('gw'))
+        timings.setdefault('gw_stream_ms', []).append(ctx.last_ms('call'))
+        timings['gw_frames'] = int((te - tb).sum())
+        timings['gw_windows'] = int(r['n_win'].sum())
+        timings['gw_dets'] = ctx.last_gw_items()
+    if r['status'] == hipabi.SPKD_ENONFINITE:
+        raise ValueError('array must not contain infs or NaNs')
+    rt = r['times']
+    n = r['n_lines']
+    line_file = owner[r['turn']]
+    bounds = np.searchsorted(line_file, np.arange(len(files) + 1))
+    _t3 = time.perf_counter()
+    cnt = np.diff(bounds)
+    kept = np.nonzero(cnt)[0]
+    seg_off = np.zeros(len(kept) + 1, dtype=np.int64)
+    seg_off[1:] = np.cumsum(cnt[kept])
+    ap = hipabi.AhcParams(cl['variant'], hipabi.KINDS[cl['kind']], cl['max_spk'], cl.get('path', 0),
+                          cl['lambdac'], cl['threshold'])
+    n_redo = len(r['redo_line'])
+    _t4 = time.perf_counter()
+    a = ctx.ahc_fused(d_frames, total_frames, r['d_seg'], r['n_ev'], r['d_index'], seg_off, r['redo_line'],
+                      r['redo_begin'], r['redo_end'], ap)
+    _t5 = time.perf_counter()
+    if timings is not None:
+        if n_redo:
+            timings.setdefault('chunk_stats', []).append(ctx.last_ms('chunk_stats'))
+            timings.setdefault('reduce_sets', []).append(ctx.last_ms('reduce_sets'))
+        timings['stats_frames'] = int((r['redo_end'] - r['redo_begin']).sum())
+        timings['stats_sets'] = n
+        timings['stats_recomputed'] = n_redo
+        for k in ('cluster_prep', 'matrix', 'ahc'):
+            timings.setdefault(k, []).append(ctx.last_ms(k))
+    if a['status'] == hipabi.SPKD_ENONFINITE:
+        raise ValueError('array must not contain infs or NaNs')
+    if timings is not None:
+        npb = np.diff(seg_off)
+        nm = a['n_merges'].astype(np.int64)
+        timings['matrix_pairs'] = int((npb * (npb - 1) // 2).sum())
+        timings['ahc_pairs'] = int((nm * (npb - 2) - nm * (nm - 1) // 2).sum())
+    if detail is not None:
+        detail['lines'] = {k: (np.array(v) if isinstance(v, np.ndarray) else v) for k, v in r.items()}
+        detail['merges'] = [list(zip(a['a'][o:o + m].tolist(), a['b'][o:o + m].tolist(), a['d'][o:o + m].tolist()))
+                            for o, m in zip(seg_off[:-1].tolist(), a['n_merges'].tolist())]
+    k0, k1 = rt[:, 0] * rate, rt[:, 1] * rate
+    in_order = (line_file[1:] != line_file[:-1]) | (k0[1:] > k0[:-1]) | ((k0[1:] == k0[:-1]) & (k1[1:] >= k1[:-1]))
+    rows = np.column_stack([rt, a['labels'].astype(np.float64)])
+    if not bool(in_order.all()):
+        rows = rows[np.lexsort((np.arange(n), k1, k0, line_file))]
+    out = [rows[bounds[i]:bounds[i + 1]] for i in range(len(files))]
+    if timings is not None:
+        _t6 = time.perf_counter()
+        timings.setdefault('wall_cd_prepare', []).append(1e3 * (_t1 - _t0))
+        timings.setdefault('wall_cd_call', []).append(1e3 * (_t2 - _t1))
+        timings.setdefault('wall_cd_finish', []).append(1e3 * (_t3 - _t2))
+        timings.setdefault('wall_cl_prepare', []).append(1e3 * (_t4 - _t3))
+        timings.setdefault('wall_cl_stats_call', []).append(0.0)
+        timings.setdefault('wall_cl_ahc_call', []).append(1e3 * (_t5 - _t4))
+        timings.setdefault('wall_cl_finish', []).append(1e3 * (_t6 - _t5))
+    return out
+
+
 def diarize_batch(ctx, d_frames, total_frames, files, rate=125.0, cd=DIA2_CD, cl=DIA2_CL, timings=None,
-                  text_contract=True, fused=False):
+                  text_contract=True, fused=False, handoff=None):
+    if handoff is None:
+        handoff = 'device' if fused and text_contract else 'host'
+    if handoff == 'device':
+        if not (fused and text_contract):
+            raise ValueError('the device hand-off is the fused mode with the text contract')
+        return diarize_batch_device(ctx, d_frames, total_frames, files, rate, cd, cl, timings)
+    if handoff != 'host':
+        raise ValueError('handoff: device or host')
     box = [] if fused else None
     segs = change_detect_batch(ctx, d_frames, total_frames, files, rate, cd, timings, text_contract, box)
     fs = box[0] if box else None
```
